# nwihardjo/SpaghettiSearch

Measured on AMD Instinct MI355X. Metric: pagerank_iters_per_sec, higher is better.
Workload: dtype f64

## Files before the change

### include/spaghetti_rank.h

```cpp
#ifndef SPAGHETTI_RANK_H
#define SPAGHETTI_RANK_H

#include <stdint.h>

#ifdef __cplusplus
extern "C" {
#endif

#define SS_ABI_VERSION 4

enum {
    SS_OK = 0,
    SS_ERR_INVALID = 1,
    SS_ERR_NO_DEVICE = 2,
    SS_ERR_HIP = 3,
    SS_ERR_OOM = 4,
    SS_ERR_UNSORTED = 5,
    SS_ERR_STATE = 6,
    SS_ERR_UNSUPPORTED = 7,
    SS_ERR_COMM = 8
};

#define SS_MAX_TOPK 1024
#define SS_MAX_TOPICS 64
#define SS_MAX_QUERY_TERMS 64
#define SS_MAX_CONSTRAINT_TERMS 16
#define SS_UNKNOWN_TERM 0xFFFFFFFFu

typedef struct ss_ctx ss_ctx;
typedef struct ss_graph ss_graph;
typedef struct ss_pr ss_pr;
typedef struct ss_index ss_index;
typedef struct ss_scorer ss_scorer;

typedef struct ss_hit {
    uint32_t doc;
    uint32_t _pad;
    double title;
    double body;
    double pagerank;
    double final;
} ss_hit;

typedef struct ss_graph_info {
    uint64_t n_nodes, n_edges;
    uint64_t n_nondangling;
    uint64_t n_rows_local;
    uint64_t n_edges_local;
    uint32_t max_indeg;
    int32_t rank, world;
} ss_graph_info;

int32_t ss_abi_version(void);
int32_t ss_init(int32_t device_id, ss_ctx** out);
int32_t ss_shutdown(ss_ctx* ctx);
int32_t ss_set_stream(ss_ctx* ctx, void* hip_stream);
int32_t ss_synchronize(ss_ctx* ctx);
#define SS_OPTION_DEFAULT INT64_MIN
int32_t ss_set_option(ss_ctx* ctx, const char* name, int64_t value);
const char* ss_last_error(ss_ctx* ctx);

#define SS_COMM_ID_BYTES 128
int32_t ss_comm_unique_id(void* id_out );
int32_t ss_comm_init(ss_ctx* ctx, const void* id , int32_t rank, int32_t world);
int32_t ss_comm_split(ss_ctx* ctx, int32_t color, int32_t key);
int32_t ss_comm_destroy(ss_ctx* ctx);
int32_t ss_comm_info(ss_ctx* ctx, int32_t* rank_out , int32_t* world_out);
int32_t ss_comm_allreduce_u64(ss_ctx* ctx, uint64_t* buf, uint64_t n);
int32_t ss_comm_allgather(ss_ctx* ctx, const void* send, void* recv, uint64_t bytes_per_rank);

int32_t ss_graph_create(ss_ctx* ctx, uint64_t n_nodes, uint64_t n_edges,
                        const uint64_t* out_ptr , const uint32_t* out_dst ,
                        int32_t rank, int32_t world, ss_graph** out);
int32_t ss_graph_apply_delta(ss_graph* g, uint64_t n_nodes_new, uint64_t n_changed, const uint32_t* changed ,
                             const uint64_t* new_ptr , const uint32_t* new_children);
int32_t ss_graph_get_info(const ss_graph* g, ss_graph_info* info);
int32_t ss_graph_destroy(ss_graph* g);

#define SS_MAX_LINKS      64
#define SS_LINKS_PARENTS  0
#define SS_LINKS_CHILDREN 1
int32_t ss_graph_set_link_key(ss_graph* g, const double* key );
int32_t ss_graph_top_links(ss_graph* g, int32_t dir, uint64_t n, const uint32_t* nodes , int32_t m,
                           uint32_t* links_out , int32_t* n_out , uint32_t* degree_out );
int32_t ss_graph_hit_links(ss_graph* g, int32_t dir, int32_t n_q, int32_t k,
                           const ss_hit* hits , const int32_t* n_hits , int32_t m,
                           uint32_t* links_out , int32_t* n_out ,
                           uint32_t* degree_out );

int32_t ss_pagerank_run(ss_graph* g, double damping, double eps, int32_t max_iter,
                        int32_t k_topics, const int32_t* n_topic,
                        double* rank_out, int32_t* iters_out);

int32_t ss_pr_create(ss_graph* g, double damping, double eps, int32_t max_iter,
                     int32_t k_topics, const int32_t* n_topic, ss_pr** out);
int32_t ss_pr_destroy(ss_pr* pr);
int32_t ss_pr_set_teleport(ss_pr* pr, const uint64_t* set_ptr , const uint32_t* set_nodes);
int32_t ss_pr_begin(ss_pr* pr);
int32_t ss_pr_step(ss_pr* pr, int32_t n_steps);
int32_t ss_pr_lean_sweeps(ss_pr* pr, int64_t* n_out);
int32_t ss_pr_finalize(ss_pr* pr);
int32_t ss_pr_exchange_buffers(ss_pr* pr, void** send_dev, uint64_t* send_bytes,
                               void** recv_dev, uint64_t* recv_bytes);
int32_t ss_pr_exchange(ss_pr* pr, int32_t allreduce);
int32_t ss_pagerank_run_sharded(ss_graph* g, double damping, double eps, int32_t max_iter, int32_t k_topics,
                                const int32_t* n_topic, int32_t allreduce, uint32_t* ids_out, double* rank_out, int32_t* iters_out);
int32_t ss_pagerank_run_group(ss_graph* const* shards, int32_t world, double damping, double eps, int32_t max_iter, int32_t k_topics,
                              const int32_t* n_topic, double* rank_out, int32_t* iters_out);
int32_t ss_pr_status(ss_pr* pr, int32_t* iters_out, int32_t* n_active, int32_t* sweeps,
                     double* last_delta_out , double* last_total_out );
int32_t ss_pr_read_local(ss_pr* pr, uint32_t* ids_out, double* rank_out);
int32_t ss_pr_read(ss_pr* pr, double* rank_out);

int32_t ss_pr_probe(ss_pr* pr, int32_t mode, int32_t n_reps, float* ms_out);

int32_t ss_index_create(ss_ctx* ctx, uint64_t n_docs, uint64_t n_terms,
                        const uint64_t* term_ptr , const uint32_t* post_doc,
                        const float* post_tf, ss_index** out);
int32_t ss_index_destroy(ss_index* idx);
int32_t ss_tfidf_build(ss_index* idx, uint64_t total_docs,
                       float* w_out, double* mag_out, float* idf_out);
int32_t ss_index_set_doc_freq(ss_index* idx, const uint64_t* df );
int32_t ss_index_set_weighted(ss_index* idx, const double* mag );
int32_t ss_index_set_positions(ss_index* idx, const uint64_t* pos_ptr, const float* pos);

int32_t ss_index_apply_delta(ss_index* idx, uint64_t n_del_docs, const uint32_t* del_docs,
                             uint64_t n_del, const uint32_t* del_term, const uint32_t* del_doc,
                             uint64_t n_add, const uint32_t* add_term, const uint32_t* add_doc, const float* add_w);
int32_t ss_index_apply_delta_pos(ss_index* idx, uint64_t n_del_docs, const uint32_t* del_docs,
                                 uint64_t n_del, const uint32_t* del_term, const uint32_t* del_doc,
                                 uint64_t n_add, const uint32_t* add_term, const uint32_t* add_doc, const float* add_w,
                                 const uint64_t* add_pos_ptr , const float* add_pos);
int32_t ss_index_resize(ss_index* idx, uint64_t n_docs_new, uint64_t n_terms_new);
int32_t ss_index_read_magnitudes(ss_index* idx, uint64_t n, const uint32_t* docs, double* mag_out);
int32_t ss_index_refresh_magnitudes(ss_index* idx, double* mag_out);
int32_t ss_index_get_info(const ss_index* idx, uint64_t* n_docs, uint64_t* n_terms, uint64_t* n_post);
int32_t ss_index_read(ss_index* idx, uint64_t* term_ptr_out , uint32_t* post_doc_out, float* post_w_out);
int32_t ss_index_read_positions(ss_index* idx, uint64_t* pos_ptr_out, float* pos_out);

int32_t ss_index_build_doc_view(ss_index* idx);
int32_t ss_index_drop_doc_view(ss_index* idx);
int32_t ss_index_read_doc_view(ss_index* idx, uint64_t* doc_ptr_out, uint32_t* doc_term_out, float* doc_w_out);
int32_t ss_index_doc_top_terms(ss_index* idx, uint64_t n, const uint32_t* docs , int32_t m,
                               uint32_t* terms_out , float* w_out , int32_t* n_out );

int32_t ss_scorer_create(ss_ctx* ctx, ss_index* title, ss_index* body, ss_scorer** out);
int32_t ss_scorer_destroy(ss_scorer* s);
int32_t ss_scorer_set_prior(ss_scorer* s, int32_t k_topics, const double* rank);
int32_t ss_score_topk(ss_scorer* s, int32_t n_q, const uint32_t* q_ptr, const uint32_t* q_terms,
                      const int32_t* query_len, const double* topic_probs, int32_t k,
                      ss_hit* hits_out, int32_t* n_hits_out);

#define SS_SCORE_INFLIGHT 3
int32_t ss_score_topk_submit(ss_scorer* s, int32_t n_q, const uint32_t* q_ptr, const uint32_t* q_terms,
                             const uint32_t* p_ptr ,
                             const uint32_t* p_terms, const int32_t* query_len, const double* topic_probs, int32_t k,
                             uint64_t* ticket_out);
int32_t ss_score_topk_collect(ss_scorer* s, uint64_t ticket, ss_hit* hits_out, int32_t* n_hits_out);

#define SS_MAX_PHRASE_TERMS 16
int32_t ss_score_topk_phrase(ss_scorer* s, int32_t n_q, const uint32_t* q_ptr, const uint32_t* q_terms,
                             const uint32_t* p_ptr, const uint32_t* p_terms, const int32_t* query_len,
                             const double* topic_probs, int32_t k, ss_hit* hits_out, int32_t* n_hits_out);

int32_t ss_scorer_set_doc_masks(ss_scorer* s, int32_t n_masks, const uint32_t* words);

int32_t ss_score_topk_masked(ss_scorer* s, int32_t n_q, const uint32_t* q_ptr, const uint32_t* q_terms,
                             const uint32_t* p_ptr, const uint32_t* p_terms, const int32_t* query_len,
                             const double* topic_probs, const int32_t* mask_id, int32_t k,
                             ss_hit* hits_out, int32_t* n_hits_out);

int32_t ss_score_topk_constrained(ss_scorer* s, int32_t n_q, const uint32_t* q_ptr, const uint32_t* q_terms,
                                  const uint32_t* p_ptr, const uint32_t* p_terms, const int32_t* query_len,
                                  const double* topic_probs, const int32_t* mask_id,
                                  const uint32_t* req_ptr , const uint32_t* req_terms,
                                  const uint32_t* exc_ptr , const uint32_t* exc_terms,
                                  int32_t k, ss_hit* hits_out, int32_t* n_hits_out);

int32_t ss_similar_topk(ss_scorer* s, int32_t n_q, const uint32_t* seeds , int32_t m,
                        const double* topic_probs, const int32_t* mask_id , int32_t k,
                        ss_hit* hits_out, int32_t* n_hits_out);

#define SS_MAX_FEEDBACK_DOCS 64
int32_t ss_related_terms(ss_scorer* s, int32_t n_q, const uint32_t* q_ptr, const uint32_t* q_terms,
                         const int32_t* query_len, const double* topic_probs, const int32_t* mask_id ,
                         int32_t k_fb, int32_t m_doc, int32_t m,
                         uint32_t* terms_out , double* score_out , int32_t* n_out );

typedef struct ss_term_match {
    float    title_w;
    float    body_w;
    uint32_t flags;
    float    body_pos;
} ss_term_match;
int32_t ss_explain_hits(ss_scorer* s, int32_t n_q, const uint32_t* q_ptr, const uint32_t* q_terms,
                        int32_t k, const ss_hit* hits , const int32_t* n_hits ,
                        int32_t t_stride, ss_term_match* out );

typedef struct ss_passage {
    float    start;
    float    last;
    uint32_t n_distinct;
    uint32_t n_occ;
    uint64_t token_mask;
} ss_passage;
int32_t ss_best_passages(ss_scorer* s, int32_t n_q, const uint32_t* q_ptr, const uint32_t* q_terms,
                         int32_t k, const ss_hit* hits , const int32_t* n_hits ,
                         int32_t width, ss_passage* out );

#define SS_NO_GROUP 0xFFFFFFFFu
int32_t ss_scorer_set_doc_groups(ss_scorer* s, const uint32_t* group );

int32_t ss_collapse_hits(ss_scorer* s, int32_t n_q, int32_t k_in, const ss_hit* hits ,
                         const int32_t* n_hits , int32_t g, int32_t first, int32_t k,
                         ss_hit* hits_out , int32_t* n_hits_out ,
                         uint32_t* same_out , int32_t* n_kept_out );

int32_t ss_score_topk_collapsed(ss_scorer* s, int32_t n_q, const uint32_t* q_ptr, const uint32_t* q_terms,
                                const int32_t* query_len, const double* topic_probs, const int32_t* mask_id ,
                                int32_t k_window, int32_t g, int32_t first, int32_t k,
                                ss_hit* hits_out , int32_t* n_hits_out ,
                                uint32_t* same_out , int32_t* n_kept_out );

#define SS_MAX_SIG_SLOTS 32
#define SS_SIG_EMPTY 0xFFFFFFFFu
int32_t ss_index_build_signatures(ss_index* idx, int32_t n_slots);
int32_t ss_index_drop_signatures(ss_index* idx);
int32_t ss_index_read_signatures(ss_index* idx, uint64_t n, const uint32_t* docs ,
                                 uint32_t* sig_out , int32_t* n_slots_out );

int32_t ss_dedup_hits(ss_scorer* s, int32_t n_q, int32_t k_in, const ss_hit* hits , const int32_t* n_hits ,
                      int32_t min_match, int32_t first, int32_t k,
                      ss_hit* hits_out , int32_t* n_hits_out ,
                      uint32_t* similar_out , int32_t* n_kept_out );

#define SS_MAX_DOC_FIELDS 4
#define SS_MAX_RANGE_CLAUSES 4
#define SS_NO_FIELD_VALUE INT64_MIN
typedef struct ss_doc_range {
    int32_t field;
    int32_t _pad;
    int64_t lo, hi;
} ss_doc_range;
int32_t ss_scorer_set_doc_fields(ss_scorer* s, int32_t n_fields, const int64_t* values );

int32_t ss_doc_field_masks(ss_scorer* s, int32_t n_sets, const uint32_t* rng_ptr , const ss_doc_range* rng,
                           const int32_t* mask_id ,
                           uint32_t* words_out );

int32_t ss_score_topk_filtered(ss_scorer* s, int32_t n_q, const uint32_t* q_ptr, const uint32_t* q_terms,
                               const uint32_t* p_ptr, const uint32_t* p_terms, const int32_t* query_len,
                               const double* topic_probs, const int32_t* mask_id,
                               const uint32_t* req_ptr , const uint32_t* req_terms,
// ... 136 lines not shown
```

### spaghettisearch_amd/_lib.py

```python
from __future__ import annotations

import ctypes as C
import os

_HERE = os.path.dirname(os.path.abspath(__file__))
LIB_PATH = os.environ.get("SS_LIB_PATH") or os.path.join(_HERE, "libspaghetti_rank.so")

SS_OK = 0
SS_MAX_TOPK = 1024
SS_MAX_TOPICS = 64
SS_MAX_QUERY_TERMS = 64
SS_MAX_FEEDBACK_DOCS = 64
SS_UNKNOWN_TERM = 0xFFFFFFFF
SS_NO_GROUP = 0xFFFFFFFF
SS_MAX_WORD_BYTES = 64
SS_MAX_EDIT_DIST = 3
SS_MAX_SUGGEST = 64
SS_MAX_COMPLETE = 64
SS_MAX_SIG_SLOTS = 32
SS_SIG_EMPTY = 0xFFFFFFFF
SS_MAX_LINKS = 64
SS_LINKS_PARENTS = 0
SS_LINKS_CHILDREN = 1
SS_MAX_DOC_FIELDS = 4
SS_MAX_RANGE_CLAUSES = 4
SS_NO_FIELD_VALUE = -(2 ** 63)
SS_MAX_VEC_DIM = 1024
SS_NO_VEC_SCORE = -(2 ** 31)
SS_DIV_WEIGHT_MAX = 65536
SS_MAX_VEC_LISTS = 65536
SS_NO_LIST = 0xFFFFFFFF
SS_FUSE_RRF = 0
SS_FUSE_WEIGHTED = 1

ERR_NAMES = {0: "SS_OK", 1: "SS_ERR_INVALID", 2: "SS_ERR_NO_DEVICE", 3: "SS_ERR_HIP", 4: "SS_ERR_OOM",
             5: "SS_ERR_UNSORTED", 6: "SS_ERR_STATE", 7: "SS_ERR_UNSUPPORTED", 8: "SS_ERR_COMM"}
SS_COMM_ID_BYTES = 128


class SpaghettiError(RuntimeError):
    def __init__(self, code: int, msg: str):
        super().__init__(f"{ERR_NAMES.get(code, code)}: {msg}")
        self.code = code


class SsHit(C.Structure):
    _fields_ = [("doc", C.c_uint32), ("_pad", C.c_uint32), ("title", C.c_double), ("body", C.c_double),
                ("pagerank", C.c_double), ("final", C.c_double)]


class SsTermMatch(C.Structure):
    _fields_ = [("title_w", C.c_float), ("body_w", C.c_float), ("flags", C.c_uint32), ("body_pos", C.c_float)]


class SsPassage(C.Structure):
    _fields_ = [("start", C.c_float), ("last", C.c_float), ("n_distinct", C.c_uint32), ("n_occ", C.c_uint32), ("token_mask", C.c_uint64)]


class SsDocRange(C.Structure):
    _fields_ = [("field", C.c_int32), ("_pad", C.c_int32), ("lo", C.c_int64), ("hi", C.c_int64)]


class SsVecHit(C.Structure):
    _fields_ = [("doc", C.c_uint32), ("score", C.c_int32)]


class SsDivInfo(C.Structure):
    _fields_ = [("rel", C.c_int32), ("sim", C.c_int32)]


class SsFuseParams(C.Structure):
    _fields_ = [("mode", C.c_int32), ("rrf_c", C.c_int32), ("w_lex", C.c_double), ("w_vec", C.c_double)]


class SsFused(C.Structure):
    _fields_ = [("score", C.c_double), ("vec_score", C.c_int32), ("lex_rank", C.c_uint16), ("vec_rank", C.c_uint16)]


class SsGraphInfo(C.Structure):
    _fields_ = [("n_nodes", C.c_uint64), ("n_edges", C.c_uint64), ("n_nondangling", C.c_uint64),
                ("n_rows_local", C.c_uint64), ("n_edges_local", C.c_uint64), ("max_indeg", C.c_uint32),
                ("rank", C.c_int32), ("world", C.c_int32)]


_vp = C.c_void_p
_i32 = C.c_int32
_u64 = C.c_uint64
_f64 = C.c_double

PROTOTYPES = {
    "ss_abi_version": (_i32, []),
    "ss_init": (_i32, [_i32, C.POINTER(_vp)]),
    "ss_shutdown": (_i32, [_vp]),
    "ss_set_stream": (_i32, [_vp, _vp]),
    "ss_synchronize": (_i32, [_vp]),
    "ss_set_option": (_i32, [_vp, C.c_char_p, C.c_int64]),
    "ss_last_error": (C.c_char_p, [_vp]),
    "ss_comm_unique_id": (_i32, [_vp]),
    "ss_comm_init": (_i32, [_vp, _vp, _i32, _i32]),
    "ss_comm_split": (_i32, [_vp, _i32, _i32]),
    "ss_comm_destroy": (_i32, [_vp]),
    "ss_comm_info": (_i32, [_vp, C.POINTER(_i32), C.POINTER(_i32)]),
    "ss_comm_allreduce_u64": (_i32, [_vp, _vp, _u64]),
    "ss_comm_allgather": (_i32, [_vp, _vp, _vp, _u64]),
    "ss_graph_create": (_i32, [_vp, _u64, _u64, _vp, _vp, _i32, _i32, C.POINTER(_vp)]),
    "ss_graph_apply_delta": (_i32, [_vp, _u64, _u64, _vp, _vp, _vp]),
    "ss_graph_get_info": (_i32, [_vp, C.POINTER(SsGraphInfo)]),
    "ss_graph_destroy": (_i32, [_vp]),
    "ss_graph_set_link_key": (_i32, [_vp, _vp]),
    "ss_graph_top_links": (_i32, [_vp, _i32, _u64, _vp, _i32, _vp, _vp, _vp]),
    "ss_graph_hit_links": (_i32, [_vp, _i32, _i32, _i32, _vp, _vp, _i32, _vp, _vp, _vp]),
    "ss_pagerank_run": (_i32, [_vp, _f64, _f64, _i32, _i32, _vp, _vp, _vp]),
    "ss_pr_create": (_i32, [_vp, _f64, _f64, _i32, _i32, _vp, C.POINTER(_vp)]),
    "ss_pr_destroy": (_i32, [_vp]),
    "ss_pr_set_teleport": (_i32, [_vp, _vp, _vp]),
    "ss_pr_begin": (_i32, [_vp]),
    "ss_pr_step": (_i32, [_vp, _i32]),
    "ss_pr_lean_sweeps": (_i32, [_vp, C.POINTER(C.c_int64)]),
    "ss_pr_finalize": (_i32, [_vp]),
    "ss_pr_exchange_buffers": (_i32, [_vp, C.POINTER(_vp), C.POINTER(_u64), C.POINTER(_vp), C.POINTER(_u64)]),
    "ss_pr_exchange": (_i32, [_vp, _i32]),
    "ss_pagerank_run_sharded": (_i32, [_vp, _f64, _f64, _i32, _i32, _vp, _i32, _vp, _vp, _vp]),
    "ss_pagerank_run_group": (_i32, [_vp, _i32, _f64, _f64, _i32, _i32, _vp, _vp, _vp]),
    "ss_pr_status": (_i32, [_vp, _vp, C.POINTER(_i32), C.POINTER(_i32), _vp, _vp]),
    "ss_pr_read_local": (_i32, [_vp, _vp, _vp]),
    "ss_pr_read": (_i32, [_vp, _vp]),
    "ss_pr_probe": (_i32, [_vp, _i32, _i32, C.POINTER(C.c_float)]),
    "ss_index_create": (_i32, [_vp, _u64, _u64, _vp, _vp, _vp, C.POINTER(_vp)]),
    "ss_index_destroy": (_i32, [_vp]),
    "ss_tfidf_build": (_i32, [_vp, _u64, _vp, _vp, _vp]),
    "ss_index_apply_delta": (_i32, [_vp, _u64, _vp, _u64, _vp, _vp, _u64, _vp, _vp, _vp]),
    "ss_index_apply_delta_pos": (_i32, [_vp, _u64, _vp, _u64, _vp, _vp, _u64, _vp, _vp, _vp, _vp, _vp]),
    "ss_index_resize": (_i32, [_vp, _u64, _u64]),
    "ss_index_read_magnitudes": (_i32, [_vp, _u64, _vp, _vp]),
    "ss_index_refresh_magnitudes": (_i32, [_vp, _vp]),
    "ss_index_get_info": (_i32, [_vp, C.POINTER(_u64), C.POINTER(_u64), C.POINTER(_u64)]),
    "ss_index_read": (_i32, [_vp, _vp, _vp, _vp]),
    "ss_index_read_positions": (_i32, [_vp, _vp, _vp]),
    "ss_index_set_doc_freq": (_i32, [_vp, _vp]),
    "ss_index_set_weighted": (_i32, [_vp, _vp]),
    "ss_index_set_positions": (_i32, [_vp, _vp, _vp]),
    "ss_index_build_doc_view": (_i32, [_vp]),
    "ss_index_drop_doc_view": (_i32, [_vp]),
    "ss_index_read_doc_view": (_i32, [_vp, _vp, _vp, _vp]),
    "ss_index_doc_top_terms": (_i32, [_vp, _u64, _vp, _i32, _vp, _vp, _vp]),
    "ss_scorer_create": (_i32, [_vp, _vp, _vp, C.POINTER(_vp)]),
    "ss_scorer_destroy": (_i32, [_vp]),
    "ss_scorer_set_prior": (_i32, [_vp, _i32, _vp]),
    "ss_score_topk": (_i32, [_vp, _i32, _vp, _vp, _vp, _vp, _i32, _vp, _vp]),
    "ss_score_topk_phrase": (_i32, [_vp, _i32, _vp, _vp, _vp, _vp, _vp, _vp, _i32, _vp, _vp]),
    "ss_score_topk_submit": (_i32, [_vp, _i32, _vp, _vp, _vp, _vp, _vp, _vp, _i32, _vp]),
    "ss_score_topk_collect": (_i32, [_vp, C.c_uint64, _vp, _vp]),
    "ss_scorer_set_doc_masks": (_i32, [_vp, _i32, _vp]),
    "ss_score_topk_masked": (_i32, [_vp, _i32, _vp, _vp, _vp, _vp, _vp, _vp, _vp, _i32, _vp, _vp]),
    "ss_score_topk_constrained": (_i32, [_vp, _i32, _vp, _vp, _vp, _vp, _vp, _vp, _vp, _vp, _vp, _vp, _vp, _i32, _vp, _vp]),
    "ss_similar_topk": (_i32, [_vp, _i32, _vp, _i32, _vp, _vp, _i32, _vp, _vp]),
    "ss_related_terms": (_i32, [_vp, _i32, _vp, _vp, _vp, _vp, _vp, _i32, _i32, _i32, _vp, _vp, _vp]),
    "ss_explain_hits": (_i32, [_vp, _i32, _vp, _vp, _i32, _vp, _vp, _i32, _vp]),
    "ss_best_passages": (_i32, [_vp, _i32, _vp, _vp, _i32, _vp, _vp, _i32, _vp]),
    "ss_scorer_set_doc_groups": (_i32, [_vp, _vp]),
    "ss_collapse_hits": (_i32, [_vp, _i32, _i32, _vp, _vp, _i32, _i32, _i32, _vp, _vp, _vp, _vp]),
    "ss_score_topk_collapsed": (_i32, [_vp, _i32, _vp, _vp, _vp, _vp, _vp, _i32, _i32, _i32, _i32, _vp, _vp, _vp, _vp]),
    "ss_index_build_signatures": (_i32, [_vp, _i32]),
    "ss_index_drop_signatures": (_i32, [_vp]),
    "ss_index_read_signatures": (_i32, [_vp, _u64, _vp, _vp, C.POINTER(_i32)]),
    "ss_dedup_hits": (_i32, [_vp, _i32, _i32, _vp, _vp, _i32, _i32, _i32, _vp, _vp, _vp, _vp]),
    "ss_scorer_set_doc_fields": (_i32, [_vp, _i32, _vp]),
    "ss_doc_field_masks": (_i32, [_vp, _i32, _vp, _vp, _vp, _vp]),
    "ss_score_topk_filtered": (_i32, [_vp, _i32, _vp, _vp, _vp, _vp, _vp, _vp, _vp, _vp, _vp, _vp, _vp, _vp, _vp, _i32, _vp, _vp]),
    "ss_facet_counts": (_i32, [_vp, _i32, _vp, _vp, _vp, _vp, _vp, _vp, _vp, _vp, _vp, _i32, _vp, _vp, _vp, _vp]),
    "ss_field_topk": (_i32, [_vp, _i32, _vp, _vp, _vp, _vp, _vp, _vp, _vp, _vp, _vp, _i32, _i32, _i32, _i32, _vp, _vp, _vp, _vp]),
    "ss_scorer_group_values": (_i32, [_vp, _vp, _vp]),
    "ss_top_groups": (_i32, [_vp, _i32, _vp, _vp, _vp, _vp, _vp, _vp, _vp, _vp, _vp, _i32, _i32, _vp, _vp, _vp, _vp, _vp]),
    "ss_sort_hits_by_field": (_i32, [_vp, _i32, _i32, _vp, _vp, _i32, _i32, _i32, _i32, _vp, _vp, _vp]),
    "ss_hit_fields": (_i32, [_vp, _i32, _i32, _vp, _vp, _vp]),
    "ss_scorer_set_doc_vectors": (_i32, [_vp, _i32, _vp]),
    "ss_vector_topk": (_i32, [_vp, _i32, _vp, _vp, _i32, _vp, _vp]),
    "ss_hit_vector_scores": (_i32, [_vp, _i32, _vp, _i32, _vp, _vp, _vp]),
    "ss_rerank_hits_by_vector": (_i32, [_vp, _i32, _vp, _i32, _vp, _vp, _i32, _i32, _vp, _vp, _vp]),
    "ss_diversify_hits": (_i32, [_vp, _i32, _vp, _i32, _vp, _vp, _i32, _i32, _i32, _i32, _vp, _vp, _vp]),
    "ss_scorer_set_vector_lists": (_i32, [_vp, _i32, _vp, _vp]),
    "ss_vector_assign_lists": (_i32, [_vp, _i32, _vp, _vp, _vp]),
    "ss_vector_topk_probed": (_i32, [_vp, _i32, _vp, _vp, _i32, _i32, _vp, _vp, _vp]),
    "ss_score_docs": (_i32, [_vp, _i32, _vp, _vp, _vp, _vp, _i32, _vp, _vp, _vp]),
    "ss_fuse_hits": (_i32, [_vp, _i32, _vp, _vp, _vp, _vp, _vp, _i32, _vp, _vp, _i32, _vp, _vp, _vp, _i32, _i32, _vp, _vp, _vp, _vp]),
    "ss_hybrid_topk": (_i32, [_vp, _i32, _vp, _vp, _vp, _vp, _vp, _vp, _i32, _vp, _i32, _i32, _vp, _vp, _vp, _vp]),
    "ss_lexicon_create": (_i32, [_vp, _u64, _vp, _vp, _vp, C.POINTER(_vp)]),
    "ss_lexicon_set_freq": (_i32, [_vp, _vp]),
    "ss_lexicon_get_info": (_i32, [_vp, C.POINTER(_u64), C.POINTER(_u64)]),
    "ss_lexicon_read_order": (_i32, [_vp, _vp]),
    "ss_lexicon_destroy": (_i32, [_vp]),
    "ss_lexicon_prefix": (_i32, [_vp, _i32, _vp, _vp, C.c_int64, _i32, _vp, _vp, _vp]),
    "ss_lexicon_suggest": (_i32, [_vp, _i32, _vp, _vp, _i32, C.c_uint32, _i32, _vp, _vp, _vp]),
    "ss_lexicon_complete": (_i32, [_vp, _i32, _vp, _vp, C.c_uint32, _i32, _vp, _vp, _vp, _vp]),
    "ss_merge_hits": (_i32, [_vp, _i32, _i32, _i32, _vp, _vp, _vp, _vp, _vp]),
    "ss_last_kernel_ms": (_i32, [_vp, _i32, C.POINTER(C.c_float)]),
}

ABI_VERSION = 4
_lib = None


def load() -> C.CDLL:
    global _lib
    if _lib is not None:
        return _lib
    if not os.path.exists(LIB_PATH):
        raise ImportError(
            f"{LIB_PATH} not found: build it with `python -c 'import __graft_entry__ as g; g.build()'` "
            "(make -C spaghettisearch_amd/csrc). There is no CPU fallback.")
    try:
        import torch
    except ImportError:
        pass
    lib = C.CDLL(LIB_PATH)
    for name, (res, args) in PROTOTYPES.items():
        fn = getattr(lib, name)
        fn.restype = res
        fn.argtypes = args
    if lib.ss_abi_version() != ABI_VERSION:
        raise ImportError(f"{LIB_PATH}: ABI version {lib.ss_abi_version()}, this binding was written for {ABI_VERSION} "
                          "(include/spaghetti_rank.h: SS_ABI_VERSION) - rebuild the library")
    _lib = lib
    return lib


def check(rc: int, ctx=None) -> None:
    if rc != SS_OK:
        msg = load().ss_last_error(ctx)
        raise SpaghettiError(rc, msg.decode("utf-8", "replace") if msg else "")
```

### spaghettisearch_amd/csrc/ctx.hip

```cpp
#include "common.hpp"
#include <chrono>

#include <unordered_map>

namespace ss {

namespace {
struct Pool {
    std::mutex mu;
    std::multimap<std::pair<int, size_t>, void*> free_blocks;
    std::unordered_map<void*, std::pair<int, size_t>> live;
    size_t held = 0, limit = (size_t)64 << 30;
    double miss_ms = 0.0;
    uint64_t misses = 0;
    int contexts = 0;
};
Pool& pool() { static Pool* p = new Pool(); return *p; }
size_t size_class(size_t b) {
    if (b <= 4096) return 4096;
    size_t p2 = 4096;
    while (p2 < b) p2 <<= 1;
    if (p2 <= ((size_t)1 << 20)) return p2;
    const size_t step = p2 >> 4;
    return (b + step - 1) / step * step;
// ... 105 lines not shown
        last = delta < 0 && pool().contexts <= 0;
    }
    if (last) pool_trim();
}

void pool_trim() {
    Pool& P = pool();
    std::multimap<std::pair<int, size_t>, void*> take;
    {
        std::lock_guard<std::mutex> lk(P.mu);
        take.swap(P.free_blocks);
        P.held = 0;
    }
    for (auto& kv : take) (void)hipFree(kv.second);
}

void pool_set_limit(size_t bytes) {
    {
        std::lock_guard<std::mutex> lk(pool().mu);
        pool().limit = bytes;
    }
    pool_trim();
}

static std::mutex g_err_mu;
static std::string g_err;
void set_global_error(const std::string& msg) {
    std::lock_guard<std::mutex> lk(g_err_mu);
    g_err = msg;
}
}

extern "C" {

int32_t ss_abi_version(void) { return SS_ABI_VERSION; }

int32_t ss_init(int32_t device_id, ss_ctx** out) {
    if (!out) {
        ss::set_global_error("ss_init: out is NULL");
        return SS_ERR_INVALID;
    }
    *out = nullptr;
    int n_dev = 0;
    hipError_t e = hipGetDeviceCount(&n_dev);
    if (e != hipSuccess || n_dev <= 0) {
        ss::set_global_error(std::string("ss_init: no HIP device (") + hipGetErrorString(e) + ")");
        return SS_ERR_NO_DEVICE;
    }
    if (device_id < 0 || device_id >= n_dev) {
        ss::set_global_error("ss_init: device_id out of range");
        return SS_ERR_INVALID;
    }
    ss_ctx* ctx = new (std::nothrow) ss_ctx();
    if (!ctx) return SS_ERR_OOM;
    ctx->device = device_id;
    if ((e = hipSetDevice(device_id)) != hipSuccess) {
        ss::set_global_error(std::string("ss_init: hipSetDevice: ") + hipGetErrorString(e));
        delete ctx;
        return SS_ERR_NO_DEVICE;
    }
    hipDeviceProp_t prop;
    if ((e = hipGetDeviceProperties(&prop, device_id)) != hipSuccess) {
        ss::set_global_error(std::string("ss_init: hipGetDeviceProperties: ") + hipGetErrorString(e));
        delete ctx;
        return SS_ERR_NO_DEVICE;
    }
    if (std::strncmp(prop.gcnArchName, "gfx950", 6) != 0) {
        ss::set_global_error(std::string("ss_init: device is ") + prop.gcnArchName +
                             ", this library is built for gfx950 (MI355X) only");
        delete ctx;
        return SS_ERR_NO_DEVICE;
    }
    ctx->cu_count = prop.multiProcessorCount;
    ctx->total_mem = prop.totalGlobalMem;
    if ((e = hipStreamCreateWithFlags(&ctx->own_stream, hipStreamNonBlocking)) != hipSuccess) {
        ss::set_global_error(std::string("ss_init: hipStreamCreate: ") + hipGetErrorString(e));
        delete ctx;
        return SS_ERR_HIP;
    }
    ctx->stream = ctx->own_stream;
    int prio_lo = 0, prio_hi = 0;
    (void)hipDeviceGetStreamPriorityRange(&prio_lo, &prio_hi);
    if ((e = hipStreamCreateWithPriority(&ctx->comm_stream, hipStreamNonBlocking, prio_hi)) != hipSuccess) {
        ss::set_global_error(std::string("ss_init: hipStreamCreate (comm): ") + hipGetErrorString(e));
        (void)hipStreamDestroy(ctx->own_stream);
        delete ctx;
        return SS_ERR_HIP;
    }
    for (int k = 0; k < 3; k++)
        for (int j = 0; j < 2; j++)
            if ((e = hipEventCreate(&ctx->ev[k][j])) != hipSuccess) {
                ss::set_global_error(std::string("ss_init: hipEventCreate: ") + hipGetErrorString(e));
                delete ctx;
                return SS_ERR_HIP;
            }
    if ((e = hipHostMalloc(reinterpret_cast<void**>(&ctx->h_pin), ss_ctx::PIN_SCRATCH, hipHostMallocDefault)) != hipSuccess) {
        ss::set_global_error(std::string("ss_init: hipHostMalloc: ") + hipGetErrorString(e));
        delete ctx;
        return SS_ERR_HIP;
    }
    ss::pool_context_count(+1);
    *out = ctx;
    return SS_OK;
}

int32_t ss_shutdown(ss_ctx* ctx) {
    if (!ctx) return SS_ERR_INVALID;
    (void)hipSetDevice(ctx->device);
    const bool stuck = !ss::try_unwedge(ctx);
    (void)ss_comm_destroy(ctx);
    if (!stuck) (void)hipStreamSynchronize(ctx->stream);
    for (int k = 0; k < 3; k++)
        for (int j = 0; j < 2; j++)
            if (ctx->ev[k][j]) (void)hipEventDestroy(ctx->ev[k][j]);
    if (ctx->comm_stream && !stuck) { (void)hipStreamSynchronize(ctx->comm_stream); (void)hipStreamDestroy(ctx->comm_stream); }
    for (hipStream_t ws : ctx->wave_stream)
        if (ws && !stuck) { (void)hipStreamSynchronize(ws); (void)hipStreamDestroy(ws); }
    if (ctx->own_stream && !stuck) (void)hipStreamDestroy(ctx->own_stream);
    if (ctx->h_pin) (void)hipHostFree(ctx->h_pin);
    for (auto& b : ctx->pin_cache) (void)hipHostFree(b.p);
    delete ctx;
    ss::pool_context_count(-1);
    return SS_OK;
}

int32_t ss_set_stream(ss_ctx* ctx, void* hip_stream) {
    if (!ctx) return SS_ERR_INVALID;
    std::lock_guard<std::recursive_mutex> lk(ctx->mu);
    SS_HIP(ctx, hipStreamSynchronize(ctx->stream));
    ctx->stream = hip_stream ? reinterpret_cast<hipStream_t>(hip_stream) : ctx->own_stream;
    return SS_OK;
}

static const char* const k_option_names[] = {
    "comm.timeout_ms",
    "pr.force_narrow",
    "pr.wire_f32",
    "pr.narrow_wave",
    "pr.t_quad",
    "pr.blocks_per_cu",
    "mem.pool_mb",
    "pr.deal_snake",
    "pr.affine_lag",
    "pr.affine",
    "pr.items_per_wave",
    "pr.persistent",
    "pr.persistent_blocks",
    "pr.n_class_order",
    "pr.class_order",
    "pr.stagger",
    "pr.deal_global",
    "pr.share_zero_rows",
    "pr.lean_sweeps",
    "pr.item_turns",
    "graph.late_free",
    "graph.readback_runs",
    "pr.trace",
    "score.collect_pinned",
    "score.pipeline_slices",
    "score.timing",
    "score.trace",
    "pr.probe_hot",
    "pr.topic_blocks",
    "tfidf.blocks",
    "tfidf.bucket_shift",
    "tfidf.head_min_run",
    "tfidf.bucket_min",
    "score.wave",
    "score.wave_max_terms",
    "score.wave_min_list",
    "score.wave_share_pct",
    "score.wave_slice_target",
    "score.wave_big_pct",
    "score.wave_big_x100",
    "score.small",
    "score.small_max_batch",
    "score.small_batch",
    "score.small_cap",
    "score.pipeline",
    "score.grade_slices",
    "score.wave_small_x100",
    "score.exact_all",
    "score.slice_target",
    "score.separate_merge",
    "passage.lds_events",
    "lexicon.chunk_terms",
    "lexicon.complete_parts",
    "links.wave_max",
    "links.chunk_edges",
    "vec.chunk_docs",
    "vec.list_seg_rows",
    "vec.list_batch_q",
    "vec.assign_batch",
    "div.scratch_bytes",
    "ftopk.runs",
    "ftopk.scratch_bytes",
    "gtopk.lds_groups",
    "gtopk.runs",
    "gtopk.scratch_bytes",
};

int32_t ss_set_option(ss_ctx* ctx, const char* name, int64_t value) {
    if (!ctx || !name) return SS_ERR_INVALID;
    std::lock_guard<std::recursive_mutex> lk(ctx->mu);
    for (const char* n : k_option_names)
        if (std::strcmp(n, name) == 0) {
            if (value == SS_OPTION_DEFAULT) ctx->options.erase(name);
            else ctx->options[name] = value;
            if (std::strcmp(name, "mem.pool_mb") == 0) ss::pool_set_limit(value == SS_OPTION_DEFAULT ? (size_t)64 << 30 : (size_t)std::max<int64_t>(0, value) << 20);
            return SS_OK;
        }
    return ctx->fail(SS_ERR_INVALID, "ss_set_option: unknown option '%s'", name);
}

int32_t ss_synchronize(ss_ctx* ctx) {
    if (!ctx) return SS_ERR_INVALID;
    std::lock_guard<std::recursive_mutex> lk(ctx->mu);
    SS_HIP(ctx, hipSetDevice(ctx->device));
    SS_TRY(ss::sync_bounded(ctx, ctx->stream, "ss_synchronize"));
    return SS_OK;
}

const char* ss_last_error(ss_ctx* ctx) {
    if (ctx) return ctx->last_error.c_str();
    static thread_local std::string tl;
    {
        std::lock_guard<std::mutex> lk(ss::g_err_mu);
        tl = ss::g_err;
    }
    return tl.c_str();
}

int32_t ss_last_kernel_ms(ss_ctx* ctx, int32_t kind, float* ms_out) {
    if (!ctx || !ms_out || kind < 0 || kind > 2) return SS_ERR_INVALID;
    std::lock_guard<std::recursive_mutex> lk(ctx->mu);
    if (!ctx->ev_valid[kind]) return ctx->fail(SS_ERR_STATE, "ss_last_kernel_ms: no timed call of kind %d yet", kind);
    SS_HIP(ctx, hipEventSynchronize(ctx->ev[kind][1]));
    SS_HIP(ctx, hipEventElapsedTime(ms_out, ctx->ev[kind][0], ctx->ev[kind][1]));
    return SS_OK;
}

}
```

### spaghettisearch_amd/csrc/pagerank.hip

```cpp
#include "pr_device.hpp"

#include <algorithm>
#include <chrono>
#include <cmath>
#include <memory>

namespace {

__global__ void k_pr_item_ranges(WorkItem* __restrict__ work, uint32_t n_items, const uint32_t* __restrict__ in_ptr) {
    const uint32_t i = blockIdx.x * blockDim.x + threadIdx.x;
    if (i >= n_items) return;
    WorkItem w = work[i];
    switch (w.kind) {
        case V_ROWW: w.beg = in_ptr[w.row]; w.end = in_ptr[w.row + 1]; break;
        case V_SEG:
            w.beg = in_ptr[w.row] + w.count * SEGW;
            w.end = min(in_ptr[w.row + 1], w.beg + SEGW);
            break;
        case V_QUAD:
        case V_DEG: w.beg = in_ptr[w.row]; w.end = in_ptr[w.row + w.count]; break;
        default: return;
    }
    work[i] = w;
}
// ... 96 lines not shown
        int owner;
        if (iid < nd_int) { owner = (int)(iid / sl_nd); lrow = (uint32_t)(iid % sl_nd); }
        else { owner = (int)((iid - nd_int) / sl_d); lrow = sl_nd + (uint32_t)((iid - nd_int) % sl_d); }
        if (owner == rank) atomicOr(&memb[lrow], 1u << k);
    }
}
__global__ void k_pr_memb_zero_count(const uint32_t* __restrict__ memb, uint32_t sl_nd, uint32_t cnt_nd, uint32_t pos_nd, uint32_t cnt_d,
                                     uint32_t pos_d, int k_topics, unsigned long long* __restrict__ cnt) {
    const uint32_t z_nd = cnt_nd - pos_nd, n_zero = z_nd + (cnt_d - pos_d);
    for (uint32_t i = blockIdx.x * blockDim.x + threadIdx.x; i < n_zero; i += gridDim.x * blockDim.x) {
        const uint32_t lrow = i < z_nd ? pos_nd + i : sl_nd + pos_d + (i - z_nd);
        const uint32_t mb = memb[lrow];
        for (int k = 0; k < k_topics; k++)
            if ((mb >> k) & 1u) atomicAdd(&cnt[k], 1ull);
    }
}

template <int GW, int POL>
__global__ __launch_bounds__(TPB) void k_pr_probe(const double* __restrict__ T, const uint32_t* __restrict__ in_src, size_t n_edges,
                                                  uint32_t n_rows, int mode, double* __restrict__ sink, uint32_t hot) {
    if constexpr (GW >= 8) {
        constexpr int NSLOT = 64 / GW;
        const int lane = threadIdx.x & 63, wave = threadIdx.x >> 6;
        const int t = lane % GW, slot = lane / GW, gbase = lane - t;
        const size_t groups = (size_t)gridDim.x * WAVES * NSLOT;
        const size_t gi = ((size_t)blockIdx.x * WAVES + wave) * NSLOT + slot;
        const size_t n_chunks = n_edges / CH;
        const size_t per = (n_chunks + groups - 1) / groups;
        size_t c = min(gi * per, n_chunks);
        const size_t c_hi = min(c + per, n_chunks);
        double acc = 0.0;
        for (; c < c_hi; c++) {
            constexpr int R = CH / GW;
            uint32_t src[R];
#pragma unroll
            for (int r = 0; r < R; r++) {
                const size_t e = c * CH + (size_t)(r * GW + t);
                uint32_t v = NT_LOAD(&in_src[e]) & SRC_MASK;
                if (mode == 1) v = (uint32_t)(((uint64_t)(v * 2654435761u + (uint32_t)e * 40503u) * n_rows) >> 32);
                if (mode == 2) v = (uint32_t)(e % n_rows);
                src[r] = v;
            }
            double v[CH];
#pragma unroll
            for (int j = 0; j < CH; j++) {
                const uint32_t sj = (uint32_t)__shfl((int)src[j / GW], gbase + (j % GW), 64);
                const double* a = &T[(size_t)sj * GW + t];
                if constexpr (POL == 0) v[j] = *a;
                else if constexpr (POL == 1) v[j] = __builtin_nontemporal_load(a);
                else if constexpr (POL == 2) v[j] = __hip_atomic_load(a, __ATOMIC_RELAXED, __HIP_MEMORY_SCOPE_AGENT);
                else if constexpr (POL == 3) v[j] = sj < hot ? *a : __builtin_nontemporal_load(a);
                else v[j] = sj < hot ? *a : __hip_atomic_load(a, __ATOMIC_RELAXED, __HIP_MEMORY_SCOPE_AGENT);
            }
#pragma unroll
            for (int j = 0; j < CH; j++) acc += v[j];
        }
        sink[((size_t)blockIdx.x * TPB + threadIdx.x)] = acc;
    }
}

}

namespace {

void pick_kernel(const ss_ctx* ctx, ss_pr* pr, int k, uint64_t table_rows) {
    const bool force_narrow = ctx->opt("pr.force_narrow", 0) != 0, narrow_wave = ctx->opt("pr.narrow_wave", 1) != 0;
    if (k > 2) {
        pr->kernel = PR_SWEEP;
        pr->gw = k <= 8 ? 8 : 16;
    } else if (force_narrow) {
        pr->kernel = PR_STEP;
        pr->gw = k;
    } else if (narrow_wave) {
        pr->kernel = PR_SWEEP_N;
        pr->gw = k;
    } else if (table_rows * 64 <= (64ull << 20)) {
        pr->kernel = PR_SWEEP;
        pr->gw = 8;
    } else {
        pr->kernel = PR_STEP;
        pr->gw = k;
    }
    pr->nwave = pr->kernel == PR_SWEEP_N;
    const int64_t want = ctx->opt("pr.persistent", 0);
    pr->persist_mode = want == 2 ? 2 : 1;
    pr->persist = pr->nwave && pr->g->world == 1 && !ctx->opt("pr.affine", 0) && want > 0;
}

template <int GW>
void launch_begin(ss_pr* pr, hipStream_t st, unsigned nb) {
    hipLaunchKernelGGL(k_pr_begin<GW>, dim3(nb), dim3(TPB), 0, st, pr->prm);
}
template <int GW>
void launch_finalize(ss_pr* pr, hipStream_t st, int is_begin) {
    hipLaunchKernelGGL(k_pr_finalize<GW>, dim3(1), dim3(64), 0, st, pr->prm, (const double*)pr->tab0.p, is_begin);
}
template <int GW>
__global__ __launch_bounds__(TPB) void k_pr_read_orig(const double* __restrict__ x, const PrCtl* __restrict__ ctl, const uint32_t* __restrict__ new_id,
                                                      uint64_t n, uint32_t sl_nd, uint32_t pos_nd, uint32_t pos_d, int k_topics,
                                                      double* __restrict__ out, const uint32_t* __restrict__ memb, uint32_t ts_mask) {
    const uint64_t v = (uint64_t)blockIdx.x * blockDim.x + threadIdx.x;
    if (v >= n) return;
    const uint32_t lrow = new_id[v];
    const bool zero = lrow < sl_nd ? lrow >= pos_nd : (lrow - sl_nd) >= pos_d;
    double r[GW];
    if (!zero) {
        if constexpr (GW >= 2) {
            const double2* const row = reinterpret_cast<const double2*>(x + (size_t)lrow * GW);
#pragma unroll
            for (int j = 0; j < GW / 2; j++) { const double2 t = row[j]; r[2 * j] = t.x; r[2 * j + 1] = t.y; }
        } else {
            r[0] = x[lrow];
        }
    } else {
        const uint32_t mb = memb ? memb[lrow] & ts_mask : 0u;
#pragma unroll
        for (int k = 0; k < GW; k++) r[k] = ((mb >> k) & 1u) ? ctl->xz_in[k] : ctl->xz[k];
    }
#pragma unroll
    for (int k = 0; k < GW; k++)
        if (k < k_topics) out[(size_t)k * n + v] = r[k];
}

template <int GW>
void launch_read(ss_pr* pr, hipStream_t st, int by_orig, uint64_t stride, uint32_t* ids, double* out) {
    const ss_graph* g = pr->g;
    const size_t n_rows = (size_t)g->cnt_nd + g->cnt_d;
    if (!n_rows) return;
    if (by_orig && g->world == 1 && !ids && stride == g->n) {
        hipLaunchKernelGGL(k_pr_read_orig<GW>, dim3(ss::div_up(g->n, TPB)), dim3(TPB), 0, st, (const double*)pr->x.p, (const PrCtl*)pr->ctl.p,
                           (const uint32_t*)g->new_id.p, g->n, g->sl_nd, pr->prm.pos_nd, pr->prm.pos_d, pr->k, out, pr->prm.memb, pr->prm.ts_mask);
        return;
    }
    hipLaunchKernelGGL(k_pr_read<GW>, dim3(ss::div_up(n_rows, TPB)), dim3(TPB), 0, st, (const double*)pr->x.p,
                       (const PrCtl*)pr->ctl.p, (const uint32_t*)g->old_id.p, g->sl_nd, g->cnt_nd, pr->prm.pos_nd, g->sl_d, g->cnt_d,
                       pr->prm.pos_d,
                       (uint64_t)g->rank * g->sl_nd, g->nd_int + (uint64_t)g->rank * g->sl_d, pr->k, stride, by_orig, ids, out,
                       pr->prm.memb, pr->prm.ts_mask);
}

#define SS_GW_DISPATCH(gw, fn, ...)          \
    switch (gw) {                            \
        case 1: fn<1>(__VA_ARGS__); break;   \
        case 2: fn<2>(__VA_ARGS__); break;   \
        case 8: fn<8>(__VA_ARGS__); break;   \
        default: fn<16>(__VA_ARGS__); break; \
    }

}

namespace ss {
unsigned begin_blocks(const ss_pr* pr) { return std::max(1u, std::min(2048u, ss::div_up((size_t)pr->g->n_local() * pr->gw, TPB))); }
void pr_launch_begin(ss_pr* pr, hipStream_t st, unsigned nb) { SS_GW_DISPATCH(pr->gw, launch_begin, pr, st, nb); }
void pr_launch_step(ss_pr* pr, hipStream_t st, bool lean) {
    switch (pr->kernel) {
        case PR_STEP: pr_step_launch(pr, st); break;
        case PR_SWEEP: pr_sweep_launch(pr, st, lean); break;
        case PR_SWEEP_N: pr_sweep_n_launch(pr, st); break;
    }
}
void pr_launch_finalize(ss_pr* pr, hipStream_t st, int is_begin) { SS_GW_DISPATCH(pr->gw, launch_finalize, pr, st, is_begin); }
}

namespace {

PlanOptions plan_options(const ss_ctx* ctx, const ss_pr* pr, size_t n_local) {
    const bool small = n_local <= ((size_t)4 << 20);
    PlanOptions o;
    o.t_quad = (uint32_t)ctx->opt("pr.t_quad", pr->nwave ? 256 : 128);
    o.item_turns = (uint32_t)std::max<int64_t>(1, std::min<int64_t>(64, ctx->opt("pr.item_turns", pr->nwave ? (small ? 1 : 4) : (small ? 4 : 8))));
    o.items_per_wave = pr->nwave ? (size_t)std::max<int64_t>(1, ctx->opt("pr.items_per_wave", 4)) : 1;
    o.deal_snake = ctx->opt("pr.deal_snake", PlanOptions::AUTO);
    o.deal_global = ctx->opt("pr.deal_global", pr->nwave && pr->gw == 1 ? 1 : 2);
    o.blocks_per_cu = ctx->opt("pr.blocks_per_cu", PlanOptions::AUTO);
    o.class_order = ctx->opt("pr.class_order", 235401);
    o.n_class_order = ctx->opt("pr.n_class_order", small ? 2310 : 123);
    o.stagger = ctx->opt("pr.stagger", 0);
    return o;
}

constexpr int OCC_MULTI_N = 3;
int blocks_per_cu(int row, int gw) {
    static std::mutex occ_mu;
    static int occ_cache[4][MAXK + 1] = {};
    std::lock_guard<std::mutex> lk_occ(occ_mu);
    int& occ = occ_cache[row][gw];
    if (!occ) {
        int per_cu = 0;
        switch (row) {
            case PR_STEP: per_cu = ss::pr_step_occupancy(gw); break;
            case PR_SWEEP: per_cu = ss::pr_sweep_occupancy(gw); break;
            case PR_SWEEP_N: per_cu = ss::pr_sweep_n_occupancy(gw); break;
            default: per_cu = ss::pr_multi_n_occupancy(gw); break;
        }
        occ = std::max(per_cu, 1);
    }
    return occ;
}
unsigned grid_for(const ss_ctx* ctx, const ss_pr* pr, const PlanOptions& opt, int per_cu, size_t n_items) {
    per_cu = (int)std::max<int64_t>(1, opt.blocks_per_cu == PlanOptions::AUTO ? per_cu : opt.blocks_per_cu);
    if (pr->persist) {
        const int admit = std::max(1, blocks_per_cu(OCC_MULTI_N, pr->gw) - 2);
        per_cu = (int)std::max<int64_t>(1, std::min<int64_t>(std::min(admit, std::max(1, per_cu / 2)), ctx->opt("pr.persistent_blocks", 4)));
    }
    return pr->kernel != PR_STEP ? (unsigned)std::min<size_t>(std::max<size_t>(1, ss::div_up(n_items, (size_t)WAVES * opt.items_per_wave)), (size_t)ctx->cu_count * per_cu)
                                 : (unsigned)std::min<size_t>(n_items, (size_t)ctx->cu_count * 8);
}

void fill_params(ss_pr* pr, const Cut& cut, const PlanOptions& opt, double damping, double eps, int32_t max_iter, int32_t k_topics) {
    const ss_graph* g = pr->g;
    PrParams& p = pr->prm;
    p.in_ptr = g->in_ptr.p;
    p.in_src = g->in_src.p;
    p.outdeg = g->outdeg.p;
    p.x = pr->x.p;
    if (g->world == 1) {
        p.tab_rd[0] = pr->tab0.p; p.tab_wr[0] = pr->tab1.p;
        p.tab_rd[1] = pr->tab1.p; p.tab_wr[1] = pr->tab0.p;
    } else {
        p.tab_rd[0] = p.tab_rd[1] = pr->tab0.p;
        p.tab_wr[0] = p.tab_wr[1] = pr->send.p;
    }
    p.work = pr->work.p;
    p.partials = pr->partials.p;
    p.segpart = pr->segpart.p;
    p.rowticket = pr->rowticket.p;
    p.hubsum = pr->hubsum.p;
    p.nmulti = cut.nmulti;
    p.ctl = pr->ctl.p;
    p.x0 = pr->x0.p;
    p.d = damping;
    p.teleport = 1.0 - damping;
    p.eps = eps;
    p.tele_n = p.teleport * (double)g->n;
    p.max_iter = max_iter;
    p.k_topics = k_topics;
    p.world = g->world;
    p.sl_nd = g->sl_nd;
    p.cnt_nd = g->cnt_nd;
    p.sl_d = g->sl_d;
    p.cnt_d = g->cnt_d;
    p.seg_edges = cut.seg_edges;
    p.n_items = (uint32_t)cut.items.size();
    p.pos_nd = cut.pos_nd;
    p.pos_d = cut.pos_d;
    p.zrow = (uint32_t)g->nd_int;
    p.tab_rows = g->sl_nd;
    p.woff = pr->woff.p;
    p.stagger_div = opt.stagger != 0 ? (uint32_t)std::max(g->ctx->cu_count, 1) : 0u;
    p.stagger_code = opt.stagger >= 10 ? (uint32_t)(opt.stagger - 10) : 0u;
    p.class_order = pack_class_order(opt.class_order);
    p.n_order = pack_n_order(opt.n_class_order);
    p.woff_lean = pr->lean ? pr->woff_lean.p : nullptr;
}

uint64_t fnv1a(const void* q, size_t n, uint64_t h = 0xcbf29ce484222325ull) {
    const unsigned char* b = static_cast<const unsigned char*>(q);
    for (size_t i = 0; i < n; i++) { h ^= b[i]; h *= 0x100000001b3ull; }
    return h;
}
void trace_plan(const ss_pr* pr, const std::vector<WorkItem>& work, const std::vector<uint32_t>& woff) {
    const PrParams& p = pr->prm;
    const double sd[] = {p.d, p.teleport, p.eps, p.tele_n};
    const uint32_t su[] = {(uint32_t)p.max_iter, (uint32_t)p.k_topics, (uint32_t)p.world, p.sl_nd, p.cnt_nd, p.sl_d, p.cnt_d, p.seg_edges, p.n_items,
                           p.pos_nd, p.pos_d, p.ts_mask, p.zrow, p.stagger_div, p.stagger_code, p.class_order, p.n_order};
    fprintf(stderr, "[pr trace] plan: work %016llx (%zu items)  woff %016llx  params %016llx  nblocks %u\n",
            (unsigned long long)fnv1a(work.data(), work.size() * sizeof(WorkItem)), work.size(),
            (unsigned long long)fnv1a(woff.data(), woff.size() * sizeof(uint32_t)),
            (unsigned long long)fnv1a(su, sizeof(su), fnv1a(sd, sizeof(sd))), pr->nblocks);
}

int32_t alloc_tables(ss_pr* pr, hipStream_t st, size_t rows) {
    const ss_graph* g = pr->g;
    ss_ctx* ctx = g->ctx;
    const size_t GW = (size_t)pr->gw;
    SS_HIP(ctx, pr->tab0.alloc(rows * GW));
    SS_HIP(ctx, hipMemsetAsync(pr->tab0.p, 0, std::max<size_t>(pr->tab0.bytes(), 8), st));
    if (g->world == 1) {
        SS_HIP(ctx, pr->tab1.alloc(rows * GW));
        SS_HIP(ctx, hipMemsetAsync(pr->tab1.p, 0, std::max<size_t>(pr->tab1.bytes(), 8), st));
    } else {
        SS_HIP(ctx, pr->send.alloc((size_t)g->sl_nd * GW));
        SS_HIP(ctx, hipMemsetAsync(pr->send.p, 0, std::max<size_t>(pr->send.bytes(), 8), st));
    }
    return SS_OK;
}
int32_t unshare_rows(ss_pr* pr, hipStream_t st) {
    if (!pr->prm.share) return SS_OK;
    const ss_graph* g = pr->g;
    SS_HIP(g->ctx, hipStreamSynchronize(st));
    SS_TRY(alloc_tables(pr, st, (size_t)g->nd_int + 1));
    pr->src_shared.release();
    pr->sh_deg.release();
    PrParams& p = pr->prm;
    p.tab_rd[0] = pr->tab0.p; p.tab_wr[0] = pr->tab1.p;
    p.tab_rd[1] = pr->tab1.p; p.tab_wr[1] = pr->tab0.p;
    p.in_src = g->in_src.p;
    p.sh_deg = nullptr;
    p.n_shared = 0;
    p.share = 0;
    p.zrow = (uint32_t)g->nd_int;
    p.tab_rows = g->sl_nd;
    return SS_OK;
}

#ifdef SS_PR_WAVETIME
void dump_wave_loads(const Cut& cut, const std::vector<double>& cost, const std::vector<uint32_t>& owner, uint32_t nw) {
    FILE* f = open_dump("pr_load.csv");
    if (!f) return;
    std::vector<double> wl(nw, 0.0), wcls((size_t)nw * 6, 0.0);
    for (size_t i = 0; i < cut.items.size(); i++) {
        int kc = 0; while (kc < 5 && i >= cut.vbeg[kc + 1]) kc++;
        wl[owner[i]] += cost[i]; wcls[(size_t)owner[i] * 6 + kc] += cost[i];
    }
    fprintf(f, "wave,load,c0,c1,c2,c3,c4,c5\n");
    for (uint32_t w = 0; w < nw; w++) fprintf(f, "%u,%.2f,%.2f,%.2f,%.2f,%.2f,%.2f,%.2f\n", w, wl[w], wcls[(size_t)w * 6], wcls[(size_t)w * 6 + 1], wcls[(size_t)w * 6 + 2], wcls[(size_t)w * 6 + 3], wcls[(size_t)w * 6 + 4], wcls[(size_t)w * 6 + 5]);
    fclose(f);
}
#endif

}

extern "C" {

int32_t ss_pr_create(ss_graph* g, double damping, double eps, int32_t max_iter, int32_t k_topics,
                     const int32_t* n_topic, ss_pr** out) {
    if (!g) return SS_ERR_INVALID;
    ss_ctx* ctx = g->ctx;
    std::lock_guard<std::recursive_mutex> lk(ctx->mu);
    if (!out) return ctx->fail(SS_ERR_INVALID, "ss_pr_create: out is NULL");
    *out = nullptr;
    if (k_topics < 1 || !n_topic) return ctx->fail(SS_ERR_INVALID, "ss_pr_create: k_topics < 1 or n_topic NULL");
    if (k_topics > MAXK) return ctx->fail(SS_ERR_UNSUPPORTED, "ss_pr_create: k_topics %d > %d per state (ss_pagerank_run splits larger K)", k_topics, MAXK);
    SS_HIP(ctx, hipSetDevice(ctx->device));
    hipStream_t st = ctx->stream;

    ss_pr* pr = new (std::nothrow) ss_pr();
    if (!pr) return ctx->fail(SS_ERR_OOM, "ss_pr_create: host OOM");
    std::unique_ptr<ss_pr> guard(pr);
    pr->g = g;
    pr->k = k_topics;
    pick_kernel(ctx, pr, k_topics, g->nd_int);
    const int GW = pr->gw;
    const bool vitems = pr->kernel != PR_STEP;
    const int GI = pr->nwave ? 8 : GW;
    const size_t n_local = g->n_local();
    if (((uint64_t)g->nd_int + 1) * GW * 8 >= (1ull << 32))
        return ctx->fail(SS_ERR_UNSUPPORTED, "ss_pr_create: contribution table of %llu rows x %d topics exceeds 4 GiB (shard the graph over more ranks)",
                         (unsigned long long)g->nd_int, GW);

    const bool trace = ctx->opt("pr.trace", 0) != 0;
    auto t_now = [] { return std::chrono::steady_clock::now(); };
    auto t_ms = [](std::chrono::steady_clock::time_point a, std::chrono::steady_clock::time_point b) { return std::chrono::duration<double, std::milli>(b - a).count(); };
    SS_HIP(ctx, pr->x.alloc(n_local * GW));
    bool share = GW >= 8 && g->world == 1 && ctx->opt("pr.affine", 0) == 0 && ctx->opt("pr.share_zero_rows", 1) != 0;
    if (!share) SS_TRY(alloc_tables(pr, st, (size_t)g->nd_int + 1));

    const auto tc0 = t_now();
    const PlanOptions opt = plan_options(ctx, pr, n_local);
    Cut cut = cut_items(g->h_indeg_nd, g->h_indeg_d, g->sl_nd, GI, pr->nwave, opt);
    const uint32_t n_tail = g->cnt_nd - cut.pos_nd;
    struct PinGuard { ss_ctx* c; void* p = nullptr; size_t cap = 0; ~PinGuard() { c->pin_free(p, cap); } } tail_od{ctx};
    if (share && n_tail == 0) {
        share = false;
        SS_TRY(alloc_tables(pr, st, (size_t)g->nd_int + 1));
    }
    if (share) {
        tail_od.p = ctx->pin_alloc((size_t)n_tail * sizeof(uint32_t), &tail_od.cap);
        if (!tail_od.p) return ctx->fail(SS_ERR_OOM, "ss_pr_create: no pinned host memory for %u out-degrees", n_tail);
        SS_HIP(ctx, hipMemcpyAsync(tail_od.p, g->outdeg.p + cut.pos_nd, (size_t)n_tail * sizeof(uint32_t), hipMemcpyDeviceToHost, st));
    }
    const auto tc1 = t_now();
    const int per_cu = blocks_per_cu(pr->kernel, GW);
    const auto tc1a = t_now();
    pr->nblocks = grid_for(ctx, pr, opt, per_cu, cut.items.size());
    static const std::vector<uint32_t> no_woff;
    const std::vector<uint32_t>* woff = &no_woff;
    if (vitems) {
        const uint32_t nw = pr->nblocks * WAVES;
        const auto td0 = t_now();
        const std::vector<double>& cost = item_costs(cut, g->h_indeg_nd, g->h_indeg_d, g->sl_nd, GI, pr->nwave);
        const auto td0a = t_now();
        std::vector<uint32_t>& owner = deal_items(cut, cost, nw, pr->nwave, opt);
#ifdef SS_PR_WAVETIME
        dump_wave_loads(cut, cost, owner, nw);
#endif
        const auto td1 = t_now();
        if (trace) fprintf(stderr, "[pr trace]   deal: occupancy query %.2f ms, costs %.3f ms, owners %.3f ms\n", t_ms(tc1, tc1a), t_ms(td0, td0a), t_ms(td0a, td1));
        woff = &place_items(cut, owner, nw);
        if (trace) fprintf(stderr, "[pr trace]   deal: placement %.3f ms\n", t_ms(td1, t_now()));
    }
    const std::vector<WorkItem>& items = cut.items;
    pr->lean = pr->kernel == PR_SWEEP && g->world == 1 && ctx->opt("pr.affine", 0) == 0 && ctx->opt("pr.lean_sweeps", 1) != 0;
    static const std::vector<WorkItem> no_items;
    const std::vector<WorkItem>* lean_items = &no_items;
    const std::vector<uint32_t>* lean_woff = &no_woff;
    if (pr->lean) {
        const auto tl0 = t_now();
        const LeanPlan lp = plan_lean_items(items, *woff, pr->nblocks * WAVES, g->sl_nd, (uint32_t)items.size());
        lean_items = &lp.items;
        lean_woff = &lp.woff;
        if (trace) fprintf(stderr, "[pr trace]   lean walk: %zu of %zu items, %.3f ms\n", lp.items.size() - 2, items.size() - 2, t_ms(tl0, t_now()));
    }

    g->settle();
    const auto tc2 = t_now();
    SharedRows sh;
    if (share) {
        SS_HIP(ctx, hipStreamSynchronize(st));
        const auto ts0 = t_now();
        sh = plan_shared_rows(static_cast<const uint32_t*>(tail_od.p), n_tail, cut.pos_nd);
        const auto ts1 = t_now();
        SS_TRY(alloc_tables(pr, st, (size_t)sh.table_rows));
        SS_HIP(ctx, pr->sh_deg.alloc(sh.deg.size()));
        SS_HIP(ctx, hipMemcpyAsync(pr->sh_deg.p, sh.deg.data(), sh.deg.size() * sizeof(uint32_t), hipMemcpyHostToDevice, st));
        SS_HIP(ctx, pr->src_shared.alloc(g->e_local));
        if (g->e_local)
            hipLaunchKernelGGL(k_pr_remap_src, dim3((unsigned)std::min<uint64_t>(ss::div_up(g->e_local, TPB), (uint64_t)ctx->cu_count * 16)), dim3(TPB), 0, st,
                               (const uint32_t*)g->in_src.p, pr->src_shared.p, (size_t)g->e_local, cut.pos_nd, g->cnt_nd, (const uint32_t*)g->outdeg.p,
                               (const uint32_t*)pr->sh_deg.p, (uint32_t)sh.deg.size(), sh.zrow);
        if (trace) fprintf(stderr, "[pr trace]   shared rows: %u rows without in-edges -> %zu shared rows (host %.3f ms), table %llu rows\n", n_tail, sh.deg.size(),
                           t_ms(ts0, ts1), (unsigned long long)sh.table_rows);
    }
    SS_HIP(ctx, pr->partials.alloc(((size_t)std::max(pr->nblocks, ss::begin_blocks(pr)) + 8) * 2 * GW));
    SS_HIP(ctx, pr->segpart.alloc((size_t)std::max(cut.nsegs, 1u) * GW));
    SS_HIP(ctx, pr->rowticket.alloc(std::max(cut.nmulti, 1u)));
    SS_HIP(ctx, pr->hubsum.alloc((size_t)std::max(cut.nmulti, 1u) * 2 * GW));
    SS_HIP(ctx, hipMemsetAsync(pr->hubsum.p, 0, pr->hubsum.bytes(), st));
    SS_HIP(ctx, hipMemsetAsync(pr->rowticket.p, 0, pr->rowticket.bytes(), st));
    SS_HIP(ctx, pr->woff.alloc(std::max<size_t>(woff->size(), 8)));
    if (!woff->empty()) SS_HIP(ctx, hipMemcpyAsync(pr->woff.p, woff->data(), woff->size() * sizeof(uint32_t), hipMemcpyHostToDevice, st));
    const size_t n_work = items.size() + lean_items->size();
    SS_HIP(ctx, pr->work.alloc(n_work));
    SS_HIP(ctx, hipMemcpyAsync(pr->work.p, items.data(), items.size() * sizeof(WorkItem), hipMemcpyHostToDevice, st));
    if (pr->lean) {
        SS_HIP(ctx, hipMemcpyAsync(pr->work.p + items.size(), lean_items->data(), lean_items->size() * sizeof(WorkItem), hipMemcpyHostToDevice, st));
        SS_HIP(ctx, pr->woff_lean.alloc(std::max<size_t>(lean_woff->size(), 8)));
        SS_HIP(ctx, hipMemcpyAsync(pr->woff_lean.p, lean_woff->data(), lean_woff->size() * sizeof(uint32_t), hipMemcpyHostToDevice, st));
    }
    if (vitems)
        hipLaunchKernelGGL(k_pr_item_ranges, dim3(ss::div_up(n_work, TPB)), dim3(TPB), 0, st, pr->work.p, (uint32_t)n_work, (const uint32_t*)g->in_ptr.p);
    SS_HIP(ctx, pr->ctl.alloc(1));
    SS_HIP(ctx, hipMemsetAsync(pr->ctl.p, 0, sizeof(PrCtl), st));
    double h_x0[MAXK];
    for (int k = 0; k < MAXK; k++) h_x0[k] = k < k_topics ? 1.0 / (double)n_topic[k] : 0.0;
    SS_HIP(ctx, pr->x0.alloc(MAXK));
    SS_HIP(ctx, hipMemcpyAsync(pr->x0.p, h_x0, sizeof(h_x0), hipMemcpyHostToDevice, st));
    SS_HIP(ctx, hipStreamSynchronize(st));
    if (trace) fprintf(stderr, "[pr trace] ss_pr_create: build_work %.2f ms (%zu items), edge ranges + deal %.2f ms, alloc + upload %.2f ms\n", t_ms(tc0, tc1), items.size(), t_ms(tc1, tc2), t_ms(tc2, t_now()));
    if (trace) fprintf(stderr, "[pr trace] where the state lives: x %p  tab0 %p  tab1 %p  in_src %p  in_ptr %p  outdeg %p  work %p  woff %p\n", (void*)pr->x.p, (void*)pr->tab0.p,
                       (void*)pr->tab1.p, (void*)g->in_src.p, (void*)g->in_ptr.p, (void*)g->outdeg.p, (void*)pr->work.p, (void*)pr->woff.p);

    fill_params(pr, cut, opt, damping, eps, max_iter, k_topics);
    if (share) {
        PrParams& p = pr->prm;
        p.in_src = pr->src_shared.p;
        p.sh_deg = pr->sh_deg.p;
        p.n_shared = (uint32_t)sh.deg.size();
        p.share = 1;
        p.zrow = sh.zrow;
        p.tab_rows = cut.pos_nd;
    }
    if (trace) trace_plan(pr, items, *woff);
    g->users++;
    *out = guard.release();
    return SS_OK;
}

int32_t ss_pr_set_teleport(ss_pr* pr, const uint64_t* set_ptr, const uint32_t* set_nodes) {
    if (!pr) return SS_ERR_INVALID;
    ss_ctx* ctx = pr->g->ctx;
    std::lock_guard<std::recursive_mutex> lk(ctx->mu);
    SS_HIP(ctx, hipSetDevice(ctx->device));
    if (pr->begun) return ctx->fail(SS_ERR_STATE, "ss_pr_set_teleport: call before ss_pr_begin");
    hipStream_t st = ctx->stream;
    PrParams& p = pr->prm;
    if (!set_ptr) {
        p.memb = nullptr; p.tin = nullptr; p.nz_in = nullptr; p.ts_mask = 0;
        return SS_OK;
    }
    const ss_graph* g = pr->g;
    const int K = pr->k;
    SS_TRY(unshare_rows(pr, st));
    std::vector<uint64_t> h_ptr(K + 1);
    SS_HIP(ctx, ss::copy_in(ctx->stream, h_ptr.data(), set_ptr, (K + 1) * sizeof(uint64_t)));
    if (h_ptr[0] != 0) return ctx->fail(SS_ERR_INVALID, "ss_pr_set_teleport: set_ptr[0] != 0");
    for (int k = 0; k < K; k++)
        if (h_ptr[k + 1] < h_ptr[k]) return ctx->fail(SS_ERR_INVALID, "ss_pr_set_teleport: set_ptr not non-decreasing");
    const uint64_t total = h_ptr[K];
    if (total && !set_nodes) return ctx->fail(SS_ERR_INVALID, "ss_pr_set_teleport: set_nodes is NULL");
    double h_tin[MAXK];
    uint32_t mask = 0;
    for (int k = 0; k < MAXK; k++) {
        h_tin[k] = 0.0;
        if (k < K && h_ptr[k + 1] > h_ptr[k]) {
            mask |= 1u << k;
            h_tin[k] = p.teleport * (double)g->n / (double)(h_ptr[k + 1] - h_ptr[k]);
        }
    }
    const size_t n_local = g->n_local();
    ss::DevBuf<uint64_t> d_ptr;
    ss::DevBuf<uint32_t> d_nodes, d_err, d_seen;
    ss::DevBuf<unsigned long long> d_cnt;
    SS_HIP(ctx, d_ptr.alloc(K + 1));
    SS_HIP(ctx, d_seen.alloc(g->n));
    SS_HIP(ctx, hipMemsetAsync(d_seen.p, 0, std::max<size_t>(d_seen.bytes(), 4), st));
    SS_HIP(ctx, d_nodes.alloc(total));
    SS_HIP(ctx, d_err.alloc(1));
    SS_HIP(ctx, d_cnt.alloc(MAXK));
    SS_HIP(ctx, pr->memb.alloc(n_local));
    SS_HIP(ctx, pr->tin.alloc(MAXK));
    SS_HIP(ctx, pr->nz_in.alloc(MAXK));
    SS_HIP(ctx, hipMemcpyAsync(d_ptr.p, h_ptr.data(), (K + 1) * sizeof(uint64_t), hipMemcpyHostToDevice, st));
    if (total) SS_HIP(ctx, hipMemcpyAsync(d_nodes.p, set_nodes, total * sizeof(uint32_t), hipMemcpyDefault, st));
    SS_HIP(ctx, hipMemsetAsync(pr->memb.p, 0, std::max<size_t>(pr->memb.bytes(), 4), st));
    SS_HIP(ctx, hipMemsetAsync(d_err.p, 0, sizeof(uint32_t), st));
    SS_HIP(ctx, hipMemsetAsync(d_cnt.p, 0, MAXK * sizeof(unsigned long long), st));
    if (total)
        hipLaunchKernelGGL(k_pr_memb, dim3(std::min<unsigned>(ss::div_up(total, TPB), 4096u)), dim3(TPB), 0, st, (const uint64_t*)d_ptr.p,
                           (const uint32_t*)d_nodes.p, K, g->n, (const uint32_t*)g->new_id.p, g->nd_int, std::max(g->sl_nd, 1u), std::max(g->sl_d, 1u),
                           g->rank, pr->memb.p, d_seen.p, d_err.p);
    const uint32_t n_zero = (g->cnt_nd - p.pos_nd) + (g->cnt_d - p.pos_d);
    if (n_zero)
        hipLaunchKernelGGL(k_pr_memb_zero_count, dim3(std::min<unsigned>(ss::div_up(n_zero, TPB), 4096u)), dim3(TPB), 0, st,
                           (const uint32_t*)pr->memb.p, g->sl_nd, g->cnt_nd, p.pos_nd, g->cnt_d, p.pos_d, K, d_cnt.p);
    SS_HIP(ctx, hipGetLastError());
    uint32_t h_err = 0;
    unsigned long long h_cnt[MAXK];
    SS_HIP(ctx, ss::fetch(ctx, st, &h_err, d_err.p, sizeof(h_err), h_cnt, d_cnt.p, sizeof(h_cnt)));
    if (h_err & 1u) return ctx->fail(SS_ERR_INVALID, "ss_pr_set_teleport: a teleport set holds a node id >= n_nodes");
    if (h_err & 2u) return ctx->fail(SS_ERR_INVALID, "ss_pr_set_teleport: a teleport set lists a node twice (the ids of a set must be distinct)");
    double h_nz[MAXK];
    for (int k = 0; k < MAXK; k++) h_nz[k] = (double)h_cnt[k];
    SS_HIP(ctx, hipMemcpyAsync(pr->tin.p, h_tin, sizeof(h_tin), hipMemcpyHostToDevice, st));
    SS_HIP(ctx, hipMemcpyAsync(pr->nz_in.p, h_nz, sizeof(h_nz), hipMemcpyHostToDevice, st));
    SS_HIP(ctx, hipStreamSynchronize(st));
    p.memb = pr->memb.p;
    p.tin = pr->tin.p;
    p.nz_in = pr->nz_in.p;
    p.ts_mask = mask;
    return SS_OK;
}

int32_t ss_pr_destroy(ss_pr* pr) {
#ifdef SS_PR_WAVETIME
    if (pr) ss::pr_dump_wave_times(pr);
#endif

    if (!pr) return SS_ERR_INVALID;
    ss_ctx* ctx = pr->g->ctx;
    std::lock_guard<std::recursive_mutex> lk(ctx->mu);
    (void)hipSetDevice(ctx->device);
    if (!ss::device_wedged(ctx->device)) {
        (void)hipStreamSynchronize(ctx->stream);
        (void)hipStreamSynchronize(ctx->comm_stream);
    }
    pr->g->users--;
    delete pr;
    return SS_OK;
}

int32_t ss_pr_begin(ss_pr* pr) {
    if (!pr) return SS_ERR_INVALID;
    ss_ctx* ctx = pr->g->ctx;
    std::lock_guard<std::recursive_mutex> lk(ctx->mu);
    SS_HIP(ctx, hipSetDevice(ctx->device));
    if (pr->need_finalize) return ctx->fail(SS_ERR_STATE, "ss_pr_begin: pending exchange/finalize");
    SS_HIP(ctx, hipMemsetAsync(&pr->ctl.p->ticket, 0, sizeof(uint32_t), ctx->stream));
    ss::pr_launch_begin(pr, ctx->stream, ss::begin_blocks(pr));
    SS_HIP(ctx, hipGetLastError());
    pr->begun = true;
    pr->sweeps_enq = 0;
    if (pr->g->world > 1) {
        pr->need_finalize = true;
        pr->finalize_is_begin = true;
    }
    return SS_OK;
}

int32_t ss_pr_step(ss_pr* pr, int32_t n_steps) {
    if (!pr) return SS_ERR_INVALID;
    return ss::pr_step(pr, n_steps, 2);
}

int32_t ss_pr_lean_sweeps(ss_pr* pr, int64_t* n_out) {
    if (!pr || !n_out) return SS_ERR_INVALID;
    std::lock_guard<std::recursive_mutex> lk(pr->g->ctx->mu);
    *n_out = pr->n_lean;
    return SS_OK;
}

}

int32_t ss::pr_step(ss_pr* pr, int32_t n_steps, int32_t full_tail) {
    ss_ctx* ctx = pr->g->ctx;
    std::lock_guard<std::recursive_mutex> lk(ctx->mu);
    SS_HIP(ctx, hipSetDevice(ctx->device));
    if (!pr->begun) return ctx->fail(SS_ERR_STATE, "ss_pr_step: ss_pr_begin not called");
    if (pr->need_finalize) return ctx->fail(SS_ERR_STATE, "ss_pr_step: pending exchange/finalize");
    if (n_steps < 1) return ctx->fail(SS_ERR_INVALID, "ss_pr_step: n_steps < 1");
    if (pr->g->world > 1 && n_steps != 1) return ctx->fail(SS_ERR_INVALID, "ss_pr_step: world>1 needs an exchange after every step");
    SS_HIP(ctx, hipEventRecord(ctx->ev[0][0], ctx->stream));
    if (pr->persist && !pr->prm.memb && !pr->prm.aff) {
        ss::pr_multi_n_launch(pr, ctx->stream, (int)n_steps);
    } else {
        const PrParams& p = pr->prm;
        const bool lean_ok = pr->lean && p.eps < 0.0 && !p.memb && !p.aff;
        for (int i = 0; i < n_steps; i++) {
            const int64_t s = pr->sweeps_enq + 1 + i;
            const bool lean = lean_ok && i + full_tail < n_steps && (p.max_iter <= 0 || s + 2 <= p.max_iter);
            ss::pr_launch_step(pr, ctx->stream, lean);
        }
    }
    pr->sweeps_enq += n_steps;
    SS_HIP(ctx, hipEventRecord(ctx->ev[0][1], ctx->stream));
    ctx->ev_valid[0] = true;
    SS_HIP(ctx, hipGetLastError());
    if (pr->g->world > 1) {
        pr->need_finalize = true;
        pr->finalize_is_begin = false;
    }
    return SS_OK;
}

extern "C" {

int32_t ss_pr_finalize(ss_pr* pr) {
    if (!pr) return SS_ERR_INVALID;
    ss_ctx* ctx = pr->g->ctx;
    std::lock_guard<std::recursive_mutex> lk(ctx->mu);
    SS_HIP(ctx, hipSetDevice(ctx->device));
    if (pr->g->world == 1) return ctx->fail(SS_ERR_STATE, "ss_pr_finalize: world==1 folds the finalize into the sweep");
    if (!pr->need_finalize) return ctx->fail(SS_ERR_STATE, "ss_pr_finalize: nothing to finalize");
    ss::pr_launch_finalize(pr, ctx->stream, pr->finalize_is_begin ? 1 : 0);
    SS_HIP(ctx, hipGetLastError());
    pr->need_finalize = false;
    return SS_OK;
}

int32_t ss_pr_exchange_buffers(ss_pr* pr, void** send_dev, uint64_t* send_bytes, void** recv_dev, uint64_t* recv_bytes) {
    if (!pr) return SS_ERR_INVALID;
    ss_ctx* ctx = pr->g->ctx;
    if (pr->g->world == 1) return ctx->fail(SS_ERR_STATE, "ss_pr_exchange_buffers: world==1 has no exchange");
    if (send_dev) *send_dev = pr->send.p;
    if (send_bytes) *send_bytes = pr->send.bytes();
    if (recv_dev) *recv_dev = pr->tab0.p;
    if (recv_bytes) *recv_bytes = (uint64_t)pr->g->nd_int * pr->gw * sizeof(double);
    return SS_OK;
}

int32_t ss_pr_exchange(ss_pr* pr, int32_t allreduce) {
    if (!pr) return SS_ERR_INVALID;
    ss_ctx* ctx = pr->g->ctx;
    std::lock_guard<std::recursive_mutex> lk(ctx->mu);
    SS_HIP(ctx, hipSetDevice(ctx->device));
    const ss_graph* g = pr->g;
    if (g->world == 1) return ctx->fail(SS_ERR_STATE, "ss_pr_exchange: world==1 has no exchange");
    if (!pr->need_finalize) return ctx->fail(SS_ERR_STATE, "ss_pr_exchange: nothing to exchange (call after ss_pr_begin / ss_pr_step)");
    if (!ctx->comm || ctx->comm_world != g->world || ctx->comm_rank != g->rank)
        return ctx->fail(SS_ERR_STATE, "ss_pr_exchange: the context's communicator (rank %d of %d) does not match the graph's shard (rank %d of %d)",
                         ctx->comm ? ctx->comm_rank : -1, ctx->comm ? ctx->comm_world : 0, g->rank, g->world);
    const size_t slice = (size_t)g->sl_nd * pr->gw;
    if (!allreduce && ctx->opt("pr.wire_f32", 0) != 0) {
        SS_HIP(ctx, ss::pr_wire_alloc(pr));
        ss::pr_wire_pack(pr, ctx->stream);
        SS_TRY(ss::comm_allgather(ctx, pr->wire_send.p, pr->wire_recv.p, ss::pr_wire_floats(pr) * sizeof(float)));
        ss::pr_wire_unpack(pr, ctx->stream);
        return SS_OK;
    }
    if (!allreduce) return ss::comm_allgather(ctx, pr->send.p, pr->tab0.p, slice * sizeof(double));
    SS_HIP(ctx, hipMemsetAsync(pr->tab0.p, 0, pr->tab0.bytes(), ctx->stream));
    SS_HIP(ctx, hipMemcpyAsync(pr->tab0.p + (size_t)g->rank * slice, pr->send.p, slice * sizeof(double), hipMemcpyDeviceToDevice, ctx->stream));
    return ss::comm_allreduce_f64(ctx, pr->tab0.p, pr->tab0.p, slice * (size_t)g->world);
}

int32_t ss_pr_status(ss_pr* pr, int32_t* iters_out, int32_t* n_active, int32_t* sweeps, double* last_delta_out,
                     double* last_total_out) {
    if (!pr) return SS_ERR_INVALID;
    ss_ctx* ctx = pr->g->ctx;
    std::lock_guard<std::recursive_mutex> lk(ctx->mu);
    SS_HIP(ctx, hipSetDevice(ctx->device));
    const PrCtl* hp = nullptr;
    SS_TRY(read_ctl(ctx, pr, ctx->stream, "ss_pr_status", &hp));
    const PrCtl h = *hp;
    if (h.stuck) return ctx->fail(SS_ERR_STATE, "ss_pr_status: the multi-sweep kernel gave up waiting between two sweeps (its grid of %u blocks was not resident: "
                                  "other kernels held the CUs for seconds); the state is void — set option pr.persistent = 0 and run again", pr->nblocks);
    for (int k = 0; k < pr->k; k++) {
        if (iters_out) iters_out[k] = h.iters[k];
        if (last_delta_out) last_delta_out[k] = h.delta[k];
        if (last_total_out) last_total_out[k] = h.S[k];
    }
    if (n_active) *n_active = h.n_active;
    if (sweeps) *sweeps = h.sweep;
    return SS_OK;
}

int32_t ss_pr_read_local(ss_pr* pr, uint32_t* ids_out, double* rank_out) {
    if (!pr || !rank_out) return SS_ERR_INVALID;
    ss_ctx* ctx = pr->g->ctx;
    std::lock_guard<std::recursive_mutex> lk(ctx->mu);
    SS_HIP(ctx, hipSetDevice(ctx->device));
    const ss_graph* g = pr->g;
    const size_t n_rows = (size_t)g->cnt_nd + g->cnt_d;
    ss::DevBuf<uint32_t> d_ids;
    ss::DevBuf<double> d_out;
    SS_HIP(ctx, d_ids.alloc(n_rows));
    SS_HIP(ctx, d_out.alloc(n_rows * pr->k));
    SS_GW_DISPATCH(pr->gw, launch_read, pr, ctx->stream, 0, (uint64_t)n_rows, d_ids.p, d_out.p);
    SS_HIP(ctx, hipGetLastError());
    if (ids_out && n_rows) SS_HIP(ctx, hipMemcpyAsync(ids_out, d_ids.p, n_rows * sizeof(uint32_t), hipMemcpyDefault, ctx->stream));
    if (n_rows) SS_HIP(ctx, hipMemcpyAsync(rank_out, d_out.p, n_rows * pr->k * sizeof(double), hipMemcpyDefault, ctx->stream));
    SS_HIP(ctx, hipStreamSynchronize(ctx->stream));
    return SS_OK;
}

int32_t ss_pr_read(ss_pr* pr, double* rank_out) {
    if (!pr || !rank_out) return SS_ERR_INVALID;
    ss_ctx* ctx = pr->g->ctx;
    std::lock_guard<std::recursive_mutex> lk(ctx->mu);
    SS_HIP(ctx, hipSetDevice(ctx->device));
    const ss_graph* g = pr->g;
    if (g->world != 1) return ctx->fail(SS_ERR_STATE, "ss_pr_read: world>1, use ss_pr_read_local");
    hipPointerAttribute_t pa{};
    const bool dev_out = hipPointerGetAttributes(&pa, rank_out) == hipSuccess && pa.type == hipMemoryTypeDevice;
    (void)hipGetLastError();
    ss::DevBuf<double> d_out;
    if (!dev_out) SS_HIP(ctx, d_out.alloc((size_t)g->n * pr->k));
    SS_GW_DISPATCH(pr->gw, launch_read, pr, ctx->stream, 1, (uint64_t)g->n, (uint32_t*)nullptr, dev_out ? rank_out : d_out.p);
    SS_HIP(ctx, hipGetLastError());
    if (!dev_out) SS_HIP(ctx, hipMemcpyAsync(rank_out, d_out.p, (size_t)g->n * pr->k * sizeof(double), hipMemcpyDefault, ctx->stream));
    SS_HIP(ctx, hipStreamSynchronize(ctx->stream));
    return SS_OK;
}

int32_t ss_pr_probe(ss_pr* pr, int32_t mode, int32_t n_reps, float* ms_out) {
    if (!pr || !ms_out) return SS_ERR_INVALID;
    ss_ctx* ctx = pr->g->ctx;
    std::lock_guard<std::recursive_mutex> lk(ctx->mu);
    SS_HIP(ctx, hipSetDevice(ctx->device));
    if (pr->gw < 8) return ctx->fail(SS_ERR_UNSUPPORTED, "ss_pr_probe: the probe mirrors the chunked gather of the K >= 5 kernels");
    if (mode < 0 || (mode & 7) > 2 || (mode >> 3) > 4 || n_reps < 1) return ctx->fail(SS_ERR_INVALID, "ss_pr_probe: mode 0..2 (+ 8 * gather cache policy 0..4), n_reps >= 1");
    const int pol = mode >> 3;
    mode &= 7;
    const uint32_t hot = (uint32_t)ctx->opt("pr.probe_hot", 24576);
    const ss_graph* g = pr->g;
    const unsigned nb = (unsigned)ctx->cu_count * 8;
    ss::DevBuf<double> sink;
    SS_HIP(ctx, sink.alloc((size_t)nb * TPB));
    hipEvent_t e0, e1;
    SS_HIP(ctx, hipEventCreate(&e0));
    SS_HIP(ctx, hipEventCreate(&e1));
    hipStream_t st = ctx->stream;
    ss::DevBuf<double> full;
    if (pr->prm.share) {
        SS_HIP(ctx, full.alloc(((size_t)g->nd_int + 1) * pr->gw));
        SS_HIP(ctx, hipMemsetAsync(full.p, 0, full.bytes(), ctx->stream));
    }
    const double* T = pr->prm.share ? full.p : pr->tab0.p;
    for (int r = 0; r < n_reps + 1; r++) {
        if (r == 1) SS_HIP(ctx, hipEventRecord(e0, st));
#define SS_PROBE_LAUNCH(GWV, POLV) hipLaunchKernelGGL((k_pr_probe<GWV, POLV>), dim3(nb), dim3(TPB), 0, st, T, (const uint32_t*)g->in_src.p, (size_t)g->e_local, (uint32_t)g->nd_int, mode, sink.p, hot)
        if (pr->gw == 8) SS_PROBE_LAUNCH(8, 0);
        else switch (pol) {
            case 0: SS_PROBE_LAUNCH(16, 0); break;
// ... 19 lines not shown
```

### spaghettisearch_amd/csrc/pr_device.hpp

```cpp
#pragma once
#include "pr_state.hpp"

#include <cmath>

namespace {


template <int GW>
__device__ __forceinline__ double wave_sum_topic(double v) {
#pragma unroll
    for (int off = GW; off < 64; off <<= 1) v += __shfl_xor(v, off, 64);
    return v;
}

__device__ __forceinline__ double zero_row_rank(const PrParams& p, int sweep, double S, double x0) {
    return ((sweep == 0 ? x0 : 0.0) + p.teleport) / S;
}
__device__ __forceinline__ double teleport_of(const PrParams& p, uint32_t lrow, int t) {
    if (!p.memb || !((p.ts_mask >> t) & 1u)) return p.teleport;
    return ((p.memb[lrow] >> t) & 1u) ? p.tin[t] : 0.0;
}
__device__ __forceinline__ double zero_row_rank_ts(const PrParams& p, int sweep, double S, double x0, double tele) {
    return ((sweep == 0 ? x0 : 0.0) + tele) / S;
}
// ... 88 lines not shown
            } else {
                const double xz = zero_row_rank(p, sw, Sk, p.x0[k]);
                ctl_st<PS>(&ctl->xz[k], xz);
                ctl_st<PS>(&ctl->xz_in[k], xz);
            }
            bool cont = dl[k] > p.eps;
            if (p.max_iter > 0 && it >= p.max_iter) cont = false;
            ctl_st<PS>(&ctl->active[k], cont ? 1 : 0);
            na += cont ? 1 : 0;
            ctl_st<PS>(&ctl->S[k], cs[k] + p.tele_n);
            ctl_st<PS>(&ctl->csum[k], cs[k]);
        }
    }
    ctl_st<PS>(&ctl->n_active, na);
    if constexpr (PS) {
        asm volatile("s_waitcnt vmcnt(0)" ::: "memory");
    }
    ctl_st<PS>(&ctl->sweep, it);
}

template <int GW, int PS = 0>
__device__ __forceinline__ void block_reduce_and_publish(const PrParams& p, double dsum, double csum, double* tail,
                                                         bool is_begin) {
    __shared__ double red[WAVES][2][MAXK];
    __shared__ double tot[2][MAXK];
    __shared__ double colsum[TPB];
    __shared__ int s_last;
    const int lane = threadIdx.x & 63, wave = threadIdx.x >> 6;
    const int t = lane % GW;
    dsum = wave_sum_topic<GW>(dsum);
    csum = wave_sum_topic<GW>(csum);
    if (lane < GW) {
        red[wave][0][t] = dsum;
        red[wave][1][t] = csum;
    }
    __syncthreads();
    if (threadIdx.x < 2 * GW) {
        const int which = threadIdx.x / GW, tt = threadIdx.x % GW;
        double v = red[0][which][tt];
#pragma unroll
        for (int w = 1; w < WAVES; w++) v += red[w][which][tt];
        __hip_atomic_store(&p.partials[(size_t)blockIdx.x * 2 * GW + threadIdx.x], v, __ATOMIC_RELAXED, __HIP_MEMORY_SCOPE_AGENT);
    }
    asm volatile("s_waitcnt vmcnt(0)" ::: "memory");
    __syncthreads();
    constexpr unsigned NG = 8;
    constexpr int NCOL = 2 * GW;
    constexpr int NPART = TPB / NCOL;
    const unsigned ng = min(NG, gridDim.x);
    const unsigned grp = blockIdx.x % ng;
    const unsigned members = (gridDim.x - grp + ng - 1) / ng;
    double* const gpart = p.partials + (size_t)gridDim.x * NCOL;
    if (threadIdx.x == 0) {
        if constexpr (PS == 2) {
            __builtin_amdgcn_fence(__ATOMIC_RELEASE, "agent");
            asm volatile("s_waitcnt vmcnt(0)" ::: "memory");
        }
        const unsigned prev = __hip_atomic_fetch_add(&p.ctl->gticket[grp], 1u, __ATOMIC_RELAXED, __HIP_MEMORY_SCOPE_AGENT);
        s_last = prev == members - 1;
    }
    __syncthreads();
    if (!s_last) return;
    const int col = threadIdx.x % NCOL, part = threadIdx.x / NCOL;
    {
        double acc = 0.0;
        for (unsigned m0 = part; m0 < members; m0 += 16 * NPART) {
            double v[16];
#pragma unroll
            for (int u = 0; u < 16; u++) {
                const unsigned m = m0 + u * NPART;
                v[u] = __hip_atomic_load(&p.partials[(size_t)(grp + ng * (m < members ? m : m0)) * NCOL + col], __ATOMIC_RELAXED, __HIP_MEMORY_SCOPE_AGENT);
            }
#pragma unroll
            for (int u = 0; u < 16; u++)
                if (m0 + u * NPART < members) acc += v[u];
        }
        colsum[threadIdx.x] = acc;
    }
    __syncthreads();
    if (threadIdx.x < NCOL) {
        double v = 0.0;
        for (int q = 0; q < NPART; q++) v += colsum[q * NCOL + threadIdx.x];
        __hip_atomic_store(&gpart[(size_t)grp * NCOL + threadIdx.x], v, __ATOMIC_RELAXED, __HIP_MEMORY_SCOPE_AGENT);
    }
    if (threadIdx.x == 0) ctl_st<PS>(&p.ctl->gticket[grp], 0u);
    asm volatile("s_waitcnt vmcnt(0)" ::: "memory");
    __syncthreads();
    if (threadIdx.x == 0) {
        const unsigned prev = __hip_atomic_fetch_add(&p.ctl->ticket, 1u, __ATOMIC_RELAXED, __HIP_MEMORY_SCOPE_AGENT);
        s_last = prev == ng - 1;
    }
    __syncthreads();
    if (!s_last) return;
    if (threadIdx.x < NCOL) {
        double v = 0.0;
        for (unsigned gq = 0; gq < ng; gq++)
            v += __hip_atomic_load(&gpart[(size_t)gq * NCOL + threadIdx.x], __ATOMIC_RELAXED, __HIP_MEMORY_SCOPE_AGENT);
        tot[threadIdx.x / GW][threadIdx.x % GW] = v;
    } else if (!is_begin && p.nmulti) {
        const unsigned hp = threadIdx.x / NCOL - 1;
        double acc = 0.0;
        for (unsigned h0 = hp; h0 < p.nmulti; h0 += 16 * (NPART - 1)) {
            double v[16];
#pragma unroll
            for (int u = 0; u < 16; u++) {
                const unsigned h = h0 + u * (NPART - 1);
                v[u] = __hip_atomic_load(&p.hubsum[(size_t)(h < p.nmulti ? h : h0) * NCOL + col], __ATOMIC_RELAXED, __HIP_MEMORY_SCOPE_AGENT);
            }
#pragma unroll
            for (int u = 0; u < 16; u++)
                if (h0 + u * (NPART - 1) < p.nmulti) acc += v[u];
        }
        colsum[threadIdx.x] = acc;
    }
    __syncthreads();
    if (!is_begin && p.nmulti && threadIdx.x < NCOL) {
        double v = tot[threadIdx.x / GW][threadIdx.x % GW];
        for (int q = 1; q < NPART; q++) v += colsum[q * NCOL + threadIdx.x];
        tot[threadIdx.x / GW][threadIdx.x % GW] = v;
    }
    __syncthreads();
    if (!is_begin && threadIdx.x < GW && ctl_ld<PS>(&p.ctl->active[threadIdx.x])) {
        const double n_zero = (double)((p.cnt_nd - p.pos_nd) + (p.cnt_d - p.pos_d));
        if (p.memb && ((p.ts_mask >> threadIdx.x) & 1u)) {
            const int k = threadIdx.x;
            const double out_new = zero_row_rank_ts(p, ctl_ld<PS>(&p.ctl->sweep), ctl_ld<PS>(&p.ctl->S[k]), p.x0[k], 0.0);
            const double in_new = zero_row_rank_ts(p, ctl_ld<PS>(&p.ctl->sweep), ctl_ld<PS>(&p.ctl->S[k]), p.x0[k], p.tin[k]);
            tot[0][k] += (n_zero - p.nz_in[k]) * fabs(out_new - ctl_ld<PS>(&p.ctl->xz[k])) + p.nz_in[k] * fabs(in_new - ctl_ld<PS>(&p.ctl->xz_in[k]));
        } else {
            const double xz_new = zero_row_rank(p, ctl_ld<PS>(&p.ctl->sweep), ctl_ld<PS>(&p.ctl->S[threadIdx.x]), p.x0[threadIdx.x]);
            tot[0][threadIdx.x] += n_zero * fabs(xz_new - ctl_ld<PS>(&p.ctl->xz[threadIdx.x]));
        }
    }
    __syncthreads();
    if (p.world == 1) {
        if (threadIdx.x == 0) {
            double dl[MAXK], cs[MAXK];
            for (int k = 0; k < MAXK; k++) {
                dl[k] = k < GW ? tot[0][k] : 0.0;
                cs[k] = k < GW ? tot[1][k] : 0.0;
            }
            ctl_st<PS>(&p.ctl->ticket, 0u);
            finalize_ctl<PS>(p, dl, cs, is_begin);
        }
    } else {
        if (threadIdx.x < GW) {
            tail[(size_t)(p.sl_nd - 2) * GW + threadIdx.x] = tot[1][threadIdx.x];
            tail[(size_t)(p.sl_nd - 1) * GW + threadIdx.x] = tot[0][threadIdx.x];
        }
        if (threadIdx.x == 0) p.ctl->ticket = 0;
    }
}

template <int GA, int GB>
__device__ __attribute__((used, noinline)) void begin_caller_context(const PrParams& p, double* tail) {
    if (!__builtin_constant_p(p.world)) return;
    block_reduce_and_publish<GA>(p, 0.0, 0.0, tail, true);
    block_reduce_and_publish<GB>(p, 0.0, 0.0, tail, true);
}

#define NT_LOAD(p) __builtin_nontemporal_load(p)
#define NT_STORE(v, p) __builtin_nontemporal_store(v, p)

constexpr uint32_t SRC_MASK = 0x7FFFFFFFu;

}
```

### spaghettisearch_amd/csrc/pr_plan.hpp

```cpp
#pragma once
#include "sorted_degrees.hpp"

#include <algorithm>
#include <cstdint>
#include <utility>
#include <vector>

namespace {

constexpr int TPB = 256;
constexpr int WAVES = TPB / 64;
constexpr int CH = 16;
constexpr uint32_t SEGW = 2048;

enum : uint32_t { W_SEG = 0, W_WAVE = 1, W_GROUP = 2, W_ZERO = 3,
                  V_SEG = 8,
                  V_ROWW = 9,
                  V_QUAD = 10,
                  V_DEG = 11,
                  V_ZERO = 12 };

struct WorkItem {
    uint32_t kind;
    uint32_t row;
// ... 200 lines not shown
    auto& load = s.load;
    auto& key = s.key;
    owner.assign(n_items, 0u);
    load.assign(nw, 0.0);
    by_load.resize(nw);
    for (uint32_t w = 0; w < nw; w++) by_load[w] = w;
    const bool snake = (opt.deal_snake == PlanOptions::AUTO ? (n_items >= (size_t)8 * nw || lane_rows ? 1 : 0) : opt.deal_snake) != 0;
    const int64_t deal_mode = opt.deal_global;
    const bool global_order = deal_mode != 0;
    if (global_order) {
        constexpr uint32_t NB = 1u << 14;
        const auto bkey = [&](size_t i) { return NB - 1 - (uint32_t)std::min<double>(cost[i] * 16.0, (double)(NB - 1)); };
        bucket.assign(NB + 1, 0u);
        order.resize(n_items);
        size_t c0 = 0;
        for (int kcls = 0; kcls < (deal_mode == 2 ? 6 : 1); kcls++) {
            const size_t c1 = deal_mode == 2 ? (kcls < 5 ? std::min<size_t>(cut.vbeg[kcls + 1], n_items) : n_items) : n_items;
            if (kcls) std::fill(bucket.begin(), bucket.end(), 0u);
            for (size_t i = c0; i < c1; i++) bucket[bkey(i) + 1]++;
            for (uint32_t b = 0; b < NB; b++) bucket[b + 1] += bucket[b];
            for (size_t i = c0; i < c1; i++) order[c0 + bucket[bkey(i)]++] = (uint32_t)i;
            c0 = c1;
        }
    }
    for (size_t i0 = 0; i0 < n_items; i0 += nw) {
        const size_t n_chunk = std::min<size_t>(nw, n_items - i0);
        if (i0 && snake) {
            std::reverse(by_load.begin(), by_load.end());
        } else if (i0) {
            key.resize(nw);
            for (uint32_t w = 0; w < nw; w++) key[w] = {load[w], w};
            std::sort(key.begin(), key.end());
            for (uint32_t w = 0; w < nw; w++) by_load[w] = key[w].second;
        }
        idx.resize(n_chunk);
        for (size_t j = 0; j < n_chunk; j++) idx[j] = global_order ? order[i0 + j] : (uint32_t)(i0 + j);
        const auto falling = [&](uint32_t a, uint32_t b) { return cost[a] > cost[b]; };
        size_t run_end = 0, n_merge = 0;
        for (size_t j = 1; j <= n_chunk && !global_order; j++) {
            if (j < n_chunk && !(cost[i0 + j] > cost[i0 + j - 1])) continue;
            if (run_end) {
                if (++n_merge > 8) { std::stable_sort(idx.begin(), idx.end(), falling); break; }
                std::inplace_merge(idx.begin(), idx.begin() + (ptrdiff_t)run_end, idx.begin() + (ptrdiff_t)j, falling);
            }
            run_end = j;
        }
        for (size_t j = 0; j < n_chunk; j++) {
            owner[idx[j]] = by_load[j];
            load[by_load[j]] += cost[idx[j]];
        }
    }
    return owner;
}

inline const std::vector<uint32_t>& place_items(Cut& cut, std::vector<uint32_t>& owner, uint32_t nw) {
    PlanScratch& s = plan_scratch();
    auto& items = cut.items;
    auto &woff = s.woff, &cnt = s.cnt;
    woff.assign((size_t)nw * 8, 0);
    cnt.assign((size_t)nw * 8, 0);
    for (int k = 0; k < 6; k++) {
        const size_t i1 = k < 5 ? std::min<size_t>(cut.vbeg[k + 1], items.size()) : items.size();
        for (size_t i = std::min<size_t>(cut.vbeg[k], i1); i < i1; i++) { owner[i] = owner[i] * 8 + (uint32_t)k; cnt[owner[i]]++; }
    }
    uint32_t run_off = 0;
    for (uint32_t w = 0; w < nw; w++) {
        for (int k = 0; k < 8; k++) {
            woff[(size_t)w * 8 + k] = run_off;
            run_off += cnt[(size_t)w * 8 + k];
            cnt[(size_t)w * 8 + k] = woff[(size_t)w * 8 + k];
        }
    }
    s.dealt.resize(items.size());
    for (size_t i = 0; i < items.size(); i++) s.dealt[cnt[owner[i]]++] = items[i];
    s.dealt.push_back({V_ZERO, 0, 0, 0, 0, 0, 0, 0});
    s.dealt.push_back({V_ZERO, 0, 0, 0, 0, 0, 0, 0});
    items.swap(s.dealt);
    return woff;
}

struct LeanPlan {
    const std::vector<WorkItem>& items;
    const std::vector<uint32_t>& woff;
};
inline LeanPlan plan_lean_items(const std::vector<WorkItem>& dealt, const std::vector<uint32_t>& woff, uint32_t nw, uint32_t sl_nd, uint32_t base) {
    PlanScratch& s = plan_scratch();
    auto& items = s.lean_items;
    auto& loff = s.lean_woff;
    items.clear();
    loff.assign((size_t)nw * 8, base);
    const size_t n = dealt.size() >= 2 ? dealt.size() - 2 : 0;
    for (size_t j = 0; j < (size_t)nw * 8 && j < woff.size(); j++) {
        loff[j] = base + (uint32_t)items.size();
        const size_t lo = std::min<size_t>(woff[j], n), hi = j + 1 < woff.size() ? std::min<size_t>(woff[j + 1], n) : n;
        for (size_t i = lo; i < hi; i++)
            if (dealt[i].row < sl_nd) items.push_back(dealt[i]);
    }
    items.push_back({V_ZERO, 0, 0, 0, 0, 0, 0, 0});
    items.push_back({V_ZERO, 0, 0, 0, 0, 0, 0, 0});
    return {items, loff};
}

inline uint32_t pack_class_order(int64_t code) {
    uint32_t packed = 0, seen = 0;
    for (int pos = 5; pos >= 0; pos--) {
        const uint32_t c = (uint32_t)(code % 10);
        code /= 10;
        packed |= (c & 7u) << (3 * pos);
        if (c < 6) seen |= 1u << c;
    }
    return seen == 0x3Fu ? packed : (0u | 1u << 3 | 2u << 6 | 3u << 9 | 4u << 12 | 5u << 15);
}
inline uint32_t pack_n_order(int64_t code) {
    uint32_t packed = 0, seen = 0;
    for (int pos = 3; pos >= 0; pos--) {
        const uint32_t c = (uint32_t)(code % 10);
        code /= 10;
        packed |= (c & 3u) << (2 * pos);
        if (c < 4) seen |= 1u << c;
    }
    return seen == 0xFu ? packed : (0u | 1u << 2 | 2u << 4 | 3u << 6);
}

struct SharedRows {
    std::vector<uint32_t> deg;
    uint32_t zrow = 0;
    uint32_t base = 0;
    uint64_t table_rows = 0;
    uint32_t row_of(uint32_t od) const {
        const auto it = std::lower_bound(deg.begin(), deg.end(), od);
        return it != deg.end() && *it == od ? base + (uint32_t)(it - deg.begin()) : zrow;
    }
};
inline SharedRows plan_shared_rows(const uint32_t* od, size_t n, uint32_t pos_nd) {
    SharedRows sh;
    uint32_t hi = 0;
    for (size_t i = 0; i < n; i++) hi = std::max(hi, od[i]);
    if (n && (uint64_t)hi <= 4 * (uint64_t)n + 65536) {
        std::vector<unsigned char> seen((size_t)hi + 1, 0);
        for (size_t i = 0; i < n; i++) seen[od[i]] = 1;
        for (size_t v = 0; v <= hi; v++)
            if (seen[v]) sh.deg.push_back((uint32_t)v);
    } else if (n) {
        sh.deg.assign(od, od + n);
        std::sort(sh.deg.begin(), sh.deg.end());
        sh.deg.erase(std::unique(sh.deg.begin(), sh.deg.end()), sh.deg.end());
    }
    sh.zrow = pos_nd;
    sh.base = pos_nd + 1;
    sh.table_rows = (uint64_t)pos_nd + 1 + sh.deg.size();
    return sh;
}

}
```

### spaghettisearch_amd/csrc/pr_state.hpp

```cpp
#pragma once
#include "graph.hpp"
#include "pr_plan.hpp"

#ifdef SS_PR_WAVETIME
#include <cstdio>
#include <cstdlib>
#include <string>
#endif

namespace {

constexpr int MAXK = 16;

struct PrCtl {
    double S[MAXK];
    double delta[MAXK];
    double csum[MAXK];
    double xz[MAXK];
    double xz_in[MAXK];
    double tele[MAXK];
    int32_t active[MAXK];
    int32_t iters[MAXK];
    int32_t sweep;
    int32_t n_active;
    uint32_t ticket;
    uint32_t stuck;
    uint32_t gticket[8];
};

constexpr int AFF_MAXK = 256;
constexpr unsigned AFF_NB = 512;
struct AffCtl {
    double u[AFF_MAXK];
    double delta[AFF_MAXK];
    int32_t active[AFF_MAXK], iters[AFF_MAXK], just[AFF_MAXK];
    double r_x, r_prev, r_next;
    double s_x, s_prev, s_next;
    double xz_prev[2];
    int32_t n_active, n_just, k_real, it;
};

struct PrParams {
    const uint32_t* in_ptr;
    const uint32_t* in_src;
    const uint32_t* outdeg;
    double* x;
    const double* tab_rd[2];
    double* tab_wr[2];
    const WorkItem* work;
    double* partials;
    double* segpart;
    uint32_t* rowticket;
    double* hubsum;
    uint32_t nmulti;
    PrCtl* ctl;
    const double* x0;
    double d, teleport, eps, tele_n;
    int32_t max_iter, k_topics, world;
    uint32_t sl_nd, cnt_nd, sl_d, cnt_d, seg_edges, n_items;
    uint32_t pos_nd, pos_d;
    const uint32_t* memb;
    const double* tin;
    const double* nz_in;
    uint32_t ts_mask;
    uint32_t zrow;
    const uint32_t* woff;
    uint32_t stagger_div;
    uint32_t stagger_code;
    uint32_t class_order;
    uint32_t n_order;
    double* x_alt;
    AffCtl* aff;
    const double* tele_col;
    const uint32_t* sh_deg;
    uint32_t n_shared;
    uint32_t share;
    uint32_t tab_rows;
    const uint32_t* woff_lean;
};

}

enum PrKernel : int {
    PR_STEP = 0,
    PR_SWEEP = 1,
    PR_SWEEP_N = 2,
};

struct ss_pr {
    ss_graph* g = nullptr;
    PrKernel kernel = PR_SWEEP;
    int gw = 1;
    ss::DevBuf<float> wire_send, wire_recv;
    bool nwave = false;
    int persist_mode = 1;
    bool persist = false;
    int k = 1;
    PrParams prm{};
    unsigned nblocks = 0;
    ss::DevBuf<double> x, tab0, tab1, send, partials, segpart, hubsum, x0;
    ss::DevBuf<uint32_t> rowticket;
    ss::DevBuf<uint32_t> memb;
    ss::DevBuf<double> tin, nz_in;
    ss::DevBuf<WorkItem> work;
    ss::DevBuf<uint32_t> woff;
    ss::DevBuf<uint32_t> src_shared;
    ss::DevBuf<uint32_t> sh_deg;
    ss::DevBuf<uint32_t> woff_lean;
    bool lean = false;
    int64_t sweeps_enq = 0;
    int64_t n_lean = 0;
    ss::DevBuf<PrCtl> ctl;
    bool begun = false;
    bool need_finalize = false;
    bool finalize_is_begin = false;
};

#pragma GCC visibility push(hidden)
namespace ss {
unsigned begin_blocks(const ss_pr* pr);
void pr_launch_begin(ss_pr* pr, hipStream_t st, unsigned nb);
void pr_launch_step(ss_pr* pr, hipStream_t st, bool lean = false);
int32_t pr_step(ss_pr* pr, int32_t n_steps, int32_t full_tail);
void pr_launch_finalize(ss_pr* pr, hipStream_t st, int is_begin);
void pr_sweep_launch(ss_pr* pr, hipStream_t st, bool lean);
int pr_sweep_occupancy(int gw);
void pr_sweep_n_launch(ss_pr* pr, hipStream_t st);
int pr_sweep_n_occupancy(int gw);
void pr_multi_n_launch(ss_pr* pr, hipStream_t st, int n_steps);
int pr_multi_n_occupancy(int gw);
void pr_step_launch(ss_pr* pr, hipStream_t st);
int pr_step_occupancy(int gw);
#ifdef SS_PR_WAVETIME
void pr_dump_wave_times(const ss_pr* pr);
#endif
size_t pr_wire_floats(const ss_pr* pr);
hipError_t pr_wire_alloc(ss_pr* pr);
void pr_wire_pack(ss_pr* pr, hipStream_t st);
void pr_wire_unpack(ss_pr* pr, hipStream_t st);
}
#pragma GCC visibility pop

namespace {
#ifdef SS_PR_WAVETIME
inline FILE* open_dump(const char* name) {
    const char* dir = getenv("SS_PR_WAVETIME_DIR");
    return fopen((std::string(dir && *dir ? dir : ".") + "/" + name).c_str(), "w");
}
#endif
inline int32_t read_ctl(ss_ctx* ctx, const ss_pr* pr, hipStream_t st, const char* what, const PrCtl** out) {
    ctx->pin_used = 0;
    PrCtl* const hp = ctx->pin<PrCtl>();
    if (hipMemcpyAsync(hp, pr->ctl.p, sizeof(PrCtl), hipMemcpyDeviceToHost, st) != hipSuccess) return ctx->fail(SS_ERR_HIP, "%s: status read failed", what);
    SS_TRY(ss::sync_bounded(ctx, st, what));
    *out = hp;
    return SS_OK;
}
}
```

### spaghettisearch_amd/csrc/pr_sweep.hip

```cpp
#include "pr_device.hpp"

#include <algorithm>

namespace {

template <int GW>
__device__ __forceinline__ double tab_at(const double* __restrict__ T, uint32_t row, int t) {
    return *reinterpret_cast<const double*>(reinterpret_cast<const char*>(T) + (size_t)((row * (uint32_t)GW + (uint32_t)t) * 8u));
}


template <int GW, bool TS, bool LEAN>
struct SweepCtx {
    const PrParams& p;
    const double* __restrict__ T;
    double* __restrict__ Tw;
    double S, x0;
    bool act;
    int t, gbase, slot;
    double dsum, csum;
};

__device__ __forceinline__ uint32_t turn_fill(uint32_t epos, uint32_t lim) {
    return min((uint32_t)CH, __builtin_elementwise_sub_sat(lim, epos));
}

template <int GW>
__device__ __forceinline__ void idx_turn(const uint32_t* __restrict__ in_src, uint32_t epos, uint32_t n, uint32_t zrow, int t, uint32_t (&src)[CH / GW]) {
#pragma unroll
    for (int r = 0; r < CH / GW; r++) {
        const uint32_t j = (uint32_t)(r * GW + t);
        const uint32_t raw = NT_LOAD(&in_src[j < n ? epos + j : 0u]);
        src[r] = j < n ? (raw & SRC_MASK) : zrow;
    }
}
template <int GW>
__device__ __forceinline__ void gather_turn(const double* __restrict__ T, const uint32_t (&src)[CH / GW], int t, int gbase, double (&v)[CH]) {
#pragma unroll
    for (int j = 0; j < CH; j++) {
        const uint32_t sj = (uint32_t)__shfl((int)src[j / GW], gbase + (j % GW), 64);
        v[j] = tab_at<GW>(T, sj, t);
    }
}

template <int GW, bool TS, bool LEAN>
__device__ __forceinline__ void finish_row(SweepCtx<GW, TS, LEAN>& c, uint32_t lrow, double y, double xo, uint32_t od, double* hub = nullptr) {
    const PrParams& p = c.p;
    y += c.x0;
    const size_t xi = (size_t)lrow * GW + c.t;
    double tele = p.teleport;
    if constexpr (TS) tele = teleport_of(p, lrow, c.t);
    double xn = (y + tele) / c.S;
    if constexpr (LEAN) {
        if (!c.act) xn = 0.0;
        const double cc = p.d * xn / (double)od;
        NT_STORE(cc, &c.Tw[xi]);
        if (hub) __hip_atomic_store(&hub[GW + c.t], cc, __ATOMIC_RELAXED, __HIP_MEMORY_SCOPE_AGENT);
        else c.csum += cc;
        return;
    }
    if (c.act) {
        NT_STORE(xn, &p.x[xi]);
        if (!hub) c.dsum += fabs(xn - xo);
    } else {
        xn = xo;
    }
    double cc = 0.0;
    if (lrow < p.sl_nd) {
        cc = p.d * xn / (double)od;
        NT_STORE(cc, &c.Tw[xi]);
        if (!hub) c.csum += cc;
    }
    if (hub) {
        __hip_atomic_store(&hub[c.t], fabs(xn - xo), __ATOMIC_RELAXED, __HIP_MEMORY_SCOPE_AGENT);
        __hip_atomic_store(&hub[GW + c.t], cc, __ATOMIC_RELAXED, __HIP_MEMORY_SCOPE_AGENT);
    }
}

template <int GW, bool TS, bool LEAN>
__device__ __forceinline__ void long_rows(SweepCtx<GW, TS, LEAN>& c, const WorkItem* __restrict__ work, uint32_t i0, uint32_t i1, int lane) {
    constexpr int NS = 64 / GW;
    constexpr uint32_t TW = NS * CH;
    const PrParams& p = c.p;
    if (i0 >= i1) return;
    WorkItem cur = work[i0], nxt = work[i0 + 1];
    uint32_t src_n[CH / GW];
    {
        const uint32_t e0 = cur.beg + (uint32_t)c.slot * CH;
        idx_turn<GW>(p.in_src, e0, turn_fill(e0, cur.end), p.zrow, c.t, src_n);
    }
    for (uint32_t it = i0; it < i1; it++) {
        const WorkItem nn = work[it + 2];
        const uint32_t lrow = cur.row;
        double xo = 0.0;
        if constexpr (!LEAN) xo = NT_LOAD(&p.x[(size_t)lrow * GW + c.t]);
        const uint32_t od = lrow < p.sl_nd ? NT_LOAD(&p.outdeg[lrow]) : 1u;
        const uint32_t turns = (cur.end - cur.beg + TW - 1) / TW;
        const bool more = it + 1 < i1;
        double acc = 0.0;
        for (uint32_t i = 0; i < turns; i++) {
            uint32_t src[CH / GW];
#pragma unroll
            for (int r = 0; r < CH / GW; r++) src[r] = src_n[r];
            const bool last = i + 1 == turns;
            const uint32_t e1 = (last ? nxt.beg : cur.beg + (i + 1) * TW) + (uint32_t)c.slot * CH;
            const uint32_t lim = last ? (more ? nxt.end : 0u) : cur.end;
            idx_turn<GW>(p.in_src, e1, turn_fill(e1, lim), p.zrow, c.t, src_n);
            double v[CH];
            gather_turn<GW>(c.T, src, c.t, c.gbase, v);
#pragma unroll
            for (int j = 0; j < CH; j++) acc += v[j];
        }
        const double y = wave_sum_topic<GW>(acc);
        if (cur.kind == V_ROWW) {
            if (lane < GW) finish_row<GW>(c, lrow, y, xo, od);
        } else {
            if (lane < GW) __hip_atomic_store(&p.segpart[(size_t)(cur.sbase + cur.count) * GW + c.t], y, __ATOMIC_RELAXED, __HIP_MEMORY_SCOPE_AGENT);
            asm volatile("s_waitcnt vmcnt(0)" ::: "memory");
            unsigned prev = 0;
            if (lane == 0) prev = __hip_atomic_fetch_add(&p.rowticket[cur.tix], 1u, __ATOMIC_RELAXED, __HIP_MEMORY_SCOPE_AGENT);
            prev = (unsigned)__builtin_amdgcn_readfirstlane((int)prev);
            if (prev == cur.nseg - 1) {
                if (lane == 0) __hip_atomic_store(&p.rowticket[cur.tix], 0u, __ATOMIC_RELAXED, __HIP_MEMORY_SCOPE_AGENT);
                if (lane < GW) {
                    double ys = 0.0;
                    for (uint32_t q = 0; q < cur.nseg; q++)
                        ys += __hip_atomic_load(&p.segpart[(size_t)(cur.sbase + q) * GW + c.t], __ATOMIC_RELAXED, __HIP_MEMORY_SCOPE_AGENT);
                    finish_row<GW>(c, lrow, ys, xo, od, p.hubsum + (size_t)cur.tix * 2 * GW);
                }
            }
        }
        cur = nxt;
        nxt = nn;
    }
}

template <int GW, bool TS, bool LEAN>
__device__ __forceinline__ void quad_rows(SweepCtx<GW, TS, LEAN>& c, const WorkItem* __restrict__ work, uint32_t i0, uint32_t i1) {
    constexpr int NS = 64 / GW;
    const PrParams& p = c.p;
    if (i0 >= i1) return;
    const uint32_t myq = (uint32_t)c.t * NS + (uint32_t)c.slot;
    auto bounds = [&](const WorkItem& w, bool live, uint32_t& bv, uint32_t& ev, uint32_t& ov) __attribute__((always_inline)) {
        const bool have = live && myq < w.count;
        const uint32_t rq = live ? w.row + (have ? myq : 0u) : 0u;
        const uint32_t b = p.in_ptr[rq], e = p.in_ptr[rq + 1];
        bv = b;
        ev = have ? e : b;
        ov = rq < p.sl_nd ? NT_LOAD(&p.outdeg[rq]) : 1u;
    };
    WorkItem cur = work[i0], nxt = work[i0 + 1];
    uint32_t cb, ce, co, nb, ne, no;
    bounds(cur, true, cb, ce, co);
    bounds(nxt, i0 + 1 < i1, nb, ne, no);
    uint32_t it = i0, q = 0, ch = 0;
    uint32_t nq = (cur.count + NS - 1) / NS, nch = cur.nseg;
    uint32_t src_n[CH / GW];
    {
        const uint32_t b0 = (uint32_t)__shfl((int)cb, c.gbase, 64), e0 = (uint32_t)__shfl((int)ce, c.gbase, 64);
        idx_turn<GW>(p.in_src, b0, turn_fill(b0, e0), p.zrow, c.t, src_n);
    }
    double acc = 0.0;
    while (it < i1) {
        uint32_t src[CH / GW];
#pragma unroll
        for (int r = 0; r < CH / GW; r++) src[r] = src_n[r];
        uint32_t qn = q, cn = ch + 1;
        bool cross = false;
        if (cn == nch) {
            cn = 0;
            qn = q + 1;
            if (qn == nq) { qn = 0; cross = true; }
        }
        const bool live_n = !cross || it + 1 < i1;
        {
            const uint32_t b_n = (uint32_t)__shfl((int)(cross ? nb : cb), c.gbase + (int)qn, 64);
            const uint32_t e_n = (uint32_t)__shfl((int)(cross ? ne : ce), c.gbase + (int)qn, 64);
            const uint32_t ep = b_n + cn * CH;
            idx_turn<GW>(p.in_src, ep, live_n ? turn_fill(ep, e_n) : 0u, p.zrow, c.t, src_n);
        }
        const bool ends = ch + 1 == nch;
        const uint32_t lrow = cur.row + q * NS + (uint32_t)c.slot;
        const bool valid = q * NS + (uint32_t)c.slot < cur.count;
        double xo = 0.0;
        if constexpr (!LEAN)
            if (ends) xo = NT_LOAD(&p.x[(size_t)(valid ? lrow : cur.row) * GW + c.t]);
        double v[CH];
        gather_turn<GW>(c.T, src, c.t, c.gbase, v);
#pragma unroll
        for (int j = 0; j < CH; j++) acc += v[j];
        if (ends) {
            const uint32_t od = (uint32_t)__shfl((int)co, c.gbase + (int)q, 64);
            if (valid) finish_row<GW>(c, lrow, acc, xo, od);
            acc = 0.0;
        }
        q = qn;
        ch = cn;
        if (cross) {
            it++;
            cur = nxt;
            cb = nb; ce = ne; co = no;
            nq = (cur.count + NS - 1) / NS;
            nch = cur.nseg;
            nxt = work[it + 1];
            bounds(nxt, it + 1 < i1, nb, ne, no);
        }
    }
}

template <int GW, int R, bool TS, bool LEAN>
__device__ __forceinline__ void deg_rows(SweepCtx<GW, TS, LEAN>& c, const WorkItem* __restrict__ work, uint32_t i0, uint32_t i1) {
    constexpr int NS = 64 / GW;
    constexpr int DM = CH / R;
    constexpr int IR = CH / GW;
    const PrParams& p = c.p;
    if (i0 >= i1) return;
    auto idx = [&](const WorkItem& w, bool live, uint32_t turn, uint32_t (&src)[IR]) __attribute__((always_inline)) {
        const uint32_t rb = (turn * NS + (uint32_t)c.slot) * R;
#pragma unroll
        for (int r = 0; r < IR; r++) {
            const uint32_t j = (uint32_t)(r * GW + c.t);
            const uint32_t rr = rb + j / DM, u = j % DM;
            const bool ok = live && u < w.nseg && rr < w.count;
            const uint32_t raw = NT_LOAD(&p.in_src[ok ? w.beg + rr * w.nseg + u : 0u]);
            src[r] = ok ? (raw & SRC_MASK) : p.zrow;
        }
    };
    WorkItem cur = work[i0], nxt = work[i0 + 1];
    uint32_t src_n[IR];
    idx(cur, true, 0, src_n);
    for (uint32_t it = i0; it < i1; it++) {
        const WorkItem nn = work[it + 2];
        const uint32_t row0 = cur.row, count = cur.count;
        const uint32_t turns = (count + NS * R - 1) / (NS * R);
        for (uint32_t i = 0; i < turns; i++) {
            uint32_t src[IR];
#pragma unroll
            for (int r = 0; r < IR; r++) src[r] = src_n[r];
            if (i + 1 < turns) idx(cur, true, i + 1, src_n);
            else idx(nxt, it + 1 < i1, 0, src_n);
            const uint32_t rb = (i * NS + (uint32_t)c.slot) * R;
            double xo[R];
#pragma unroll
            for (int r = 0; r < R; r++) {
                xo[r] = 0.0;
                if constexpr (!LEAN) xo[r] = NT_LOAD(&p.x[(size_t)(row0 + (rb + r < count ? rb + r : 0u)) * GW + c.t]);
            }
            const uint32_t myr = row0 + (rb + (uint32_t)c.t < count ? rb + (uint32_t)c.t : 0u);
            const uint32_t odv = (c.t < R && myr < p.sl_nd) ? NT_LOAD(&p.outdeg[myr]) : 1u;
            double v[CH];
            gather_turn<GW>(c.T, src, c.t, c.gbase, v);
#pragma unroll
            for (int r = 0; r < R; r++) {
                double y = 0.0;
#pragma unroll
                for (int u = 0; u < DM; u++) y += v[r * DM + u];
                const uint32_t od = (uint32_t)__shfl((int)odv, c.gbase + r, 64);
                if (rb + r < count) finish_row<GW>(c, row0 + rb + r, y, xo[r], od);
            }
        }
        cur = nxt;
        nxt = nn;
    }
}

#ifndef SS_PR_MINW
#define SS_PR_MINW 1
#endif
#ifdef SS_PR_WAVETIME
__device__ unsigned long long g_pr_wt[65536][2];
#endif
template <int GW, bool TS, bool LEAN>
__global__ __launch_bounds__(TPB, SS_PR_MINW) void k_pr_sweep(PrParams p) {
    static_assert(!(TS && LEAN), "the lean sweep exists without teleport sets only");
    constexpr int NS = 64 / GW;
    PrCtl* ctl = p.ctl;
    if (ctl->n_active == 0) return;
#ifdef SS_PR_WAVETIME
    unsigned long long wt0;
    asm volatile("s_memrealtime %0\n\ts_waitcnt lgkmcnt(0)" : "=s"(wt0));
#endif
    const int sweep = ctl->sweep;
    const int lane = threadIdx.x & 63;
    const uint32_t wave = (uint32_t)__builtin_amdgcn_readfirstlane((int)(threadIdx.x >> 6));
    SweepCtx<GW, TS, LEAN> c{p, p.tab_rd[sweep & 1], p.tab_wr[sweep & 1], 0.0, 0.0, false, lane % GW, lane - lane % GW, lane / GW, 0.0, 0.0};
    c.S = ctl->S[c.t];
    c.act = ctl->active[c.t] != 0;
    c.x0 = sweep == 0 ? p.x0[c.t] : 0.0;

    if constexpr (!TS) {
        if (p.n_shared) {
            const double xz_out = c.act ? zero_row_rank(p, sweep, c.S, p.x0[c.t]) : ctl->xz[c.t];
            const uint32_t nel = p.n_shared * (uint32_t)GW;
            for (uint32_t i = blockIdx.x * TPB + threadIdx.x; i < nel; i += gridDim.x * TPB)
                c.Tw[(size_t)(p.zrow + 1) * GW + i] = p.d * xz_out / (double)p.sh_deg[i / GW];
        }
    }

    const uint32_t* __restrict__ off = (LEAN ? p.woff_lean : p.woff) + (size_t)(blockIdx.x * WAVES + wave) * 8;
    int rot = p.stagger_div ? (int)((blockIdx.x / p.stagger_div) % 6u) : 0;
    if (p.stagger_code) {
        uint32_t cdv = p.stagger_code;
        for (uint32_t r = blockIdx.x / p.stagger_div; r > 0; r--) cdv /= 6u;
        rot = (int)(cdv % 6u);
    }
    for (int s6 = 0; s6 < 6; s6++) {
    const int cls = (int)((p.class_order >> (3 * ((s6 + rot) % 6))) & 7u);
    {
        int ln = lane;
        asm volatile("" : "+v"(ln));
        c.t = ln % GW;
        c.gbase = ln - ln % GW;
        c.slot = ln / GW;
    }
    switch (cls) {
    case 0: long_rows<GW>(c, p.work, off[0], off[1], lane); break;
    case 1: quad_rows<GW>(c, p.work, off[1], off[2]); break;
    case 2: deg_rows<GW, 2>(c, p.work, off[2], off[3]); break;
    case 3: deg_rows<GW, 4>(c, p.work, off[3], off[4]); break;
    case 4: deg_rows<GW, 8>(c, p.work, off[4], off[5]); break;
    default:
    for (uint32_t item = off[5]; item < off[6]; item++) {
        const WorkItem w = p.work[item];
        const bool store = TS || !p.share;
        const bool ts = TS && p.memb && ((p.ts_mask >> c.t) & 1u);
        const double xz_out = c.act ? (ts ? zero_row_rank_ts(p, sweep, c.S, p.x0[c.t], 0.0) : zero_row_rank(p, sweep, c.S, p.x0[c.t])) : ctl->xz[c.t];
        const double xz_inn = ts ? (c.act ? zero_row_rank_ts(p, sweep, c.S, p.x0[c.t], p.tin[c.t]) : ctl->xz_in[c.t]) : xz_out;
        uint32_t od[16];
#pragma unroll
        for (int i = 0; i < 16; i++) {
            const uint32_t rr = (uint32_t)(i * NS + c.slot);
            od[i] = NT_LOAD(&p.outdeg[w.row + (rr < w.count ? rr : 0u)]);
        }
#pragma unroll
        for (int i = 0; i < 16; i++) {
            const uint32_t rr = (uint32_t)(i * NS + c.slot);
            if (rr < w.count) {
                const uint32_t lrow = w.row + rr;
                const double xz = ts && ((p.memb[lrow] >> c.t) & 1u) ? xz_inn : xz_out;
                const double cc = p.d * xz / (double)od[i];
                if (store) NT_STORE(cc, &c.Tw[(size_t)lrow * GW + c.t]);
                c.csum += cc;
            }
        }
    }
    break;
    }
    }
#ifdef SS_PR_WAVETIME
    {
        unsigned long long wt1;
        asm volatile("s_waitcnt vmcnt(0)\n\ts_memrealtime %0\n\ts_waitcnt lgkmcnt(0)" : "=s"(wt1));
        const uint32_t wid = (blockIdx.x * WAVES + wave) & 65535u;
        if (lane == 0) { g_pr_wt[wid][0] = wt0; g_pr_wt[wid][1] = wt1; }
    }
#endif
    block_reduce_and_publish<GW>(p, LEAN ? 0.0 : c.dsum, c.csum, c.Tw, false);
}

template __device__ void begin_caller_context<8, 16>(const PrParams&, double*);

}

namespace ss {
void pr_sweep_launch(ss_pr* pr, hipStream_t st, bool lean) {
    const bool ts = pr->prm.memb != nullptr;
    lean = lean && !ts && pr->prm.woff_lean;
    if (lean) pr->n_lean++;
    if (pr->gw == 8) {
        if (ts) hipLaunchKernelGGL((k_pr_sweep<8, true, false>), dim3(pr->nblocks), dim3(TPB), 0, st, pr->prm);
        else if (lean) hipLaunchKernelGGL((k_pr_sweep<8, false, true>), dim3(pr->nblocks), dim3(TPB), 0, st, pr->prm);
        else hipLaunchKernelGGL((k_pr_sweep<8, false, false>), dim3(pr->nblocks), dim3(TPB), 0, st, pr->prm);
    } else {
        if (ts) hipLaunchKernelGGL((k_pr_sweep<16, true, false>), dim3(pr->nblocks), dim3(TPB), 0, st, pr->prm);
        else if (lean) hipLaunchKernelGGL((k_pr_sweep<16, false, true>), dim3(pr->nblocks), dim3(TPB), 0, st, pr->prm);
        else hipLaunchKernelGGL((k_pr_sweep<16, false, false>), dim3(pr->nblocks), dim3(TPB), 0, st, pr->prm);
    }
}
int pr_sweep_occupancy(int gw) {
    int per_cu = 8;
    if (gw == 8) (void)hipOccupancyMaxActiveBlocksPerMultiprocessor(&per_cu, k_pr_sweep<8, false, false>, TPB, 0);
    else (void)hipOccupancyMaxActiveBlocksPerMultiprocessor(&per_cu, k_pr_sweep<16, false, false>, TPB, 0);
    return per_cu;
}

#ifdef SS_PR_WAVETIME
void pr_dump_wave_times(const ss_pr* pr) {
    if (pr->gw < 8) return;
    (void)hipDeviceSynchronize();
    const uint32_t nwv = std::min<uint32_t>(65536u, pr->nblocks * WAVES);
    std::vector<unsigned long long> h((size_t)nwv * 2);
    if (hipMemcpyFromSymbol(h.data(), HIP_SYMBOL(g_pr_wt), h.size() * sizeof(unsigned long long)) != hipSuccess || !nwv) return;
    unsigned long long t0 = ~0ull;
    for (uint32_t w = 0; w < nwv; w++) t0 = std::min(t0, h[2 * w]);
    std::vector<double> st(nwv), en(nwv);
    for (uint32_t w = 0; w < nwv; w++) { st[w] = (double)(h[2 * w] - t0) / 100.0; en[w] = (double)(h[2 * w + 1] - t0) / 100.0; }
    std::sort(st.begin(), st.end()); std::sort(en.begin(), en.end());
    if (FILE* f = open_dump("pr_wt.csv")) {
        fprintf(f, "wave,start_us,end_us\n");
        for (uint32_t w = 0; w < nwv; w++) fprintf(f, "%u,%.2f,%.2f\n", w, (double)(h[2 * w] - t0) / 100.0, (double)(h[2 * w + 1] - t0) / 100.0);
        fclose(f);
    }
    fprintf(stderr, "[pr wavetime] %u waves: start us median %.1f max %.1f | out of items us min %.1f p10 %.1f median %.1f p90 %.1f p99 %.1f max %.1f\n", nwv,
            st[nwv / 2], st[nwv - 1], en[0], en[nwv / 10], en[nwv / 2], en[nwv * 9 / 10], en[(size_t)nwv * 99 / 100], en[nwv - 1]);
}
#endif
}
```

### spaghettisearch_amd/engine.py

```python
from __future__ import annotations

import ctypes as C
from typing import Optional, Sequence

import numpy as np

from . import _lib
from ._lib import SsGraphInfo, SsHit, SsPassage, SsTermMatch, check

HIT_DTYPE = np.dtype([("doc", "<u4"), ("_pad", "<u4"), ("title", "<f8"), ("body", "<f8"),
                      ("pagerank", "<f8"), ("final", "<f8")])

TERM_MATCH_DTYPE = np.dtype([("title_w", "<f4"), ("body_w", "<f4"), ("flags", "<u4"), ("body_pos", "<f4")])

PASSAGE_DTYPE = np.dtype([("start", "<f4"), ("last", "<f4"), ("n_distinct", "<u4"), ("n_occ", "<u4"), ("token_mask", "<u8")])

DOC_RANGE_DTYPE = np.dtype([("field", "<i4"), ("_pad", "<i4"), ("lo", "<i8"), ("hi", "<i8")])

VEC_HIT_DTYPE = np.dtype([("doc", "<u4"), ("score", "<i4")])

GROUP_COUNT_DTYPE = np.dtype([("group", "<u4"), ("count", "<u4")])

DIV_INFO_DTYPE = np.dtype([("rel", "<i4"), ("sim", "<i4")])

# ... 159 lines not shown
    def apply_delta(self, n_nodes_new: int, changed, new_ptr, new_children) -> None:
        changed = _as(changed, "uint32")
        new_ptr = _as(new_ptr, "uint64")
        new_children = _as(new_children, "uint32")
        self.ctx.ready(changed, new_ptr, new_children)
        check(self.ctx.lib.ss_graph_apply_delta(self.h, int(n_nodes_new), int(changed.shape[0]), _ptr(changed), _ptr(new_ptr), _ptr(new_children)),
              self.ctx.h)
        self.n = int(n_nodes_new)

    def info(self) -> SsGraphInfo:
        gi = SsGraphInfo()
        check(self.ctx.lib.ss_graph_get_info(self.h, C.byref(gi)), self.ctx.h)
        return gi

    def pagerank_sharded(self, damping: float, eps: float, n_topic: Sequence[int], max_iter: int = 0, allreduce: bool = False, out=None):
        n_topic = np.ascontiguousarray(np.atleast_1d(n_topic), dtype=np.int32)
        K = len(n_topic)
        rows = int(self.info().n_rows_local)
        if out is not None:
            ids, rank = _as(out[0], "uint32"), _as(out[1], "float64")
            count = lambda a: a.numel() if _is_torch(a) else a.size
            if count(ids) < rows or count(rank) < K * rows:
                raise ValueError("out arrays too small")
        else:
            ids = np.zeros(rows, dtype=np.uint32)
            rank = np.zeros((K, rows), dtype=np.float64)
        iters = np.zeros(K, dtype=np.int32)
        check(self.ctx.lib.ss_pagerank_run_sharded(self.h, damping, eps, max_iter, K, _ptr(n_topic), 1 if allreduce else 0,
                                                   _ptr(ids), _ptr(rank), _ptr(iters)), self.ctx.h)
        return ids, rank, iters

    def pagerank(self, damping: float, eps: float, n_topic: Sequence[int], max_iter: int = 0):
        n_topic = np.ascontiguousarray(np.atleast_1d(n_topic), dtype=np.int32)
        K = len(n_topic)
        rank = np.zeros((K, self.n), dtype=np.float64)
        iters = np.zeros(K, dtype=np.int32)
        check(self.ctx.lib.ss_pagerank_run(self.h, damping, eps, max_iter, K, _ptr(n_topic), _ptr(rank), _ptr(iters)),
              self.ctx.h)
        return rank, iters

    @staticmethod
    def pagerank_group(shards, damping: float, eps: float, n_topic: Sequence[int], max_iter: int = 0):
        n_topic = np.ascontiguousarray(np.atleast_1d(n_topic), dtype=np.int32)
        K = len(n_topic)
        ctx = shards[0].ctx
        hs = (C.c_void_p * len(shards))(*[g.h for g in shards])
        rank = np.zeros((K, shards[0].n), dtype=np.float64)
        iters = np.zeros(K, dtype=np.int32)
        check(ctx.lib.ss_pagerank_run_group(hs, len(shards), damping, eps, max_iter, K, _ptr(n_topic), _ptr(rank), _ptr(iters)), ctx.h)
        return rank, iters

    def pagerank_dev(self, damping: float, eps: float, n_topic: Sequence[int], rank_out, max_iter: int = 0):
        n_topic = np.ascontiguousarray(np.atleast_1d(n_topic), dtype=np.int32)
        K = len(n_topic)
        rank_out = _as(rank_out, "float64")
        if rank_out.numel() < K * self.n:
            raise ValueError("rank_out too small")
        iters = np.zeros(K, dtype=np.int32)
        check(self.ctx.lib.ss_pagerank_run(self.h, damping, eps, max_iter, K, _ptr(n_topic), _ptr(rank_out), _ptr(iters)),
              self.ctx.h)
        return iters

    def set_link_key(self, key) -> None:
        if key is None:
            check(self.ctx.lib.ss_graph_set_link_key(self.h, None), self.ctx.h)
            return
        key = _as(key, "float64")
        if (key.numel() if _is_torch(key) else key.size) < self.n:
            raise ValueError("key must hold n_nodes values")
        self.ctx.ready(key)
        check(self.ctx.lib.ss_graph_set_link_key(self.h, _ptr(key)), self.ctx.h)

    def _links_out(self, rows: int, m: int, want_degree: bool, out):
        count = lambda a: a.numel() if _is_torch(a) else a.size
        if out is not None:
            links, n_out, degree = _as(out[0], "uint32"), _as(out[1], "int32"), _as(out[2], "uint32") if len(out) > 2 else None
            if count(links) < rows * m or count(n_out) < rows or (degree is not None and count(degree) < rows):
                raise ValueError("output buffers too small")
            return links, n_out, degree
        return np.zeros(rows * m, dtype=np.uint32), np.zeros(rows, dtype=np.int32), np.zeros(rows, dtype=np.uint32) if want_degree else None

    def top_links(self, nodes, direction: int, m: int = 5, want_degree: bool = True, out=None):
        nodes = _as(nodes, "uint32")
        n = int(nodes.numel() if _is_torch(nodes) else nodes.size)
        links, n_out, degree = self._links_out(n, int(m), want_degree, out)
        self.ctx.ready(nodes, links, n_out, degree)
        check(self.ctx.lib.ss_graph_top_links(self.h, int(direction), n, _ptr(nodes), int(m), _ptr(links), _ptr(n_out), _ptr(degree)), self.ctx.h)
        if out is None:
            links = links.reshape(n, int(m))
        elif any(_is_torch(a) for a in (links, n_out, degree)) and not getattr(self.ctx, "_shared_stream", False):
            self.ctx.synchronize()
        return links, n_out, degree

    def hit_links(self, hits, n_hits, direction: int, m: int = 5, want_degree: bool = True, out=None, k: Optional[int] = None):
        n_hits = _as(n_hits, "int32")
        n_q = int(n_hits.numel() if _is_torch(n_hits) else n_hits.size)
        nbytes = lambda a: a.numel() * a.element_size() if _is_torch(a) else a.nbytes
        hits = hits.contiguous() if _is_torch(hits) else np.ascontiguousarray(hits, dtype=HIT_DTYPE)
        if k is None:
            if n_q > 0 and nbytes(hits) % (n_q * HIT_DTYPE.itemsize):
                raise ValueError("hits does not hold n_q rows of whole ss_hit")
            k = nbytes(hits) // (n_q * HIT_DTYPE.itemsize) if n_q > 0 else 1
        elif nbytes(hits) < n_q * int(k) * HIT_DTYPE.itemsize:
            raise ValueError("hits too small")
        k = int(k)
        links, n_out, degree = self._links_out(n_q * k, int(m), want_degree, out)
        self.ctx.ready(hits, n_hits, links, n_out, degree)
        check(self.ctx.lib.ss_graph_hit_links(self.h, int(direction), n_q, k, _ptr(hits), _ptr(n_hits), int(m), _ptr(links), _ptr(n_out),
                                              _ptr(degree)), self.ctx.h)
        if out is None:
            links, n_out = links.reshape(n_q, k, int(m)), n_out.reshape(n_q, k)
            degree = degree.reshape(n_q, k) if degree is not None else None
        elif any(_is_torch(a) for a in (links, n_out, degree)) and not getattr(self.ctx, "_shared_stream", False):
            self.ctx.synchronize()
        return links, n_out, degree

    def close(self) -> None:
        if self.h:
            self.ctx.lib.ss_graph_destroy(self.h)
            self.h = None


class PageRankState:

    def __init__(self, graph: Graph, damping: float, eps: float, n_topic: Sequence[int], max_iter: int = 0):
        self.g = graph
        self.ctx = graph.ctx
        n_topic = np.ascontiguousarray(np.atleast_1d(n_topic), dtype=np.int32)
        self.k = len(n_topic)
        h = C.c_void_p()
        check(self.ctx.lib.ss_pr_create(graph.h, damping, eps, max_iter, self.k, _ptr(n_topic), C.byref(h)), self.ctx.h)
        self.h = h

    def set_teleport(self, sets) -> None:
        if sets is None:
            check(self.ctx.lib.ss_pr_set_teleport(self.h, None, None), self.ctx.h)
            return
        if len(sets) != self.k:
            raise ValueError("one teleport set per topic")
        ptr = np.zeros(self.k + 1, dtype=np.uint64)
        ptr[1:] = np.cumsum([len(x) for x in sets])
        nodes = np.ascontiguousarray(np.concatenate([np.asarray(x, dtype=np.uint32) for x in sets]) if int(ptr[-1]) else np.zeros(0, np.uint32))
        check(self.ctx.lib.ss_pr_set_teleport(self.h, _ptr(ptr), _ptr(nodes)), self.ctx.h)

    def begin(self) -> None:
        check(self.ctx.lib.ss_pr_begin(self.h), self.ctx.h)

    def step(self, n_steps: int = 1) -> None:
        check(self.ctx.lib.ss_pr_step(self.h, n_steps), self.ctx.h)

    def lean_sweeps(self) -> int:
        n = C.c_int64(0)
        check(self.ctx.lib.ss_pr_lean_sweeps(self.h, C.byref(n)), self.ctx.h)
        return int(n.value)

    def finalize(self) -> None:
        check(self.ctx.lib.ss_pr_finalize(self.h), self.ctx.h)

    def exchange(self, allreduce: bool = False) -> None:
        check(self.ctx.lib.ss_pr_exchange(self.h, 1 if allreduce else 0), self.ctx.h)

    def exchange_buffers(self):
        sp, rp = C.c_void_p(), C.c_void_p()
        sb, rb = C.c_uint64(), C.c_uint64()
        check(self.ctx.lib.ss_pr_exchange_buffers(self.h, C.byref(sp), C.byref(sb), C.byref(rp), C.byref(rb)), self.ctx.h)
        return sp.value, sb.value, rp.value, rb.value

    def status(self):
        iters = np.zeros(self.k, dtype=np.int32)
        delta = np.zeros(self.k, dtype=np.float64)
        total = np.zeros(self.k, dtype=np.float64)
        na, sw = C.c_int32(), C.c_int32()
        check(self.ctx.lib.ss_pr_status(self.h, _ptr(iters), C.byref(na), C.byref(sw), _ptr(delta), _ptr(total)), self.ctx.h)
        return {"iters": iters, "n_active": na.value, "sweeps": sw.value, "delta": delta, "total": total}

    def probe(self, mode: int = 0, n_reps: int = 5) -> float:
        ms = C.c_float(0)
        check(self.ctx.lib.ss_pr_probe(self.h, mode, n_reps, C.byref(ms)), self.ctx.h)
        return float(ms.value)

    def read(self) -> np.ndarray:
        out = np.zeros((self.k, self.g.n), dtype=np.float64)
        check(self.ctx.lib.ss_pr_read(self.h, _ptr(out)), self.ctx.h)
        return out

    def read_local(self):
        n_rows = int(self.g.info().n_rows_local)
        ids = np.zeros(n_rows, dtype=np.uint32)
        out = np.zeros((self.k, n_rows), dtype=np.float64)
        check(self.ctx.lib.ss_pr_read_local(self.h, _ptr(ids), _ptr(out)), self.ctx.h)
        return ids, out

    def close(self) -> None:
        if self.h:
            self.ctx.lib.ss_pr_destroy(self.h)
            self.h = None


class InvertedIndex:

    def __init__(self, ctx: Context, n_docs: int, term_ptr, post_doc, post_tf):
        self.ctx = ctx
        self.n_docs = int(n_docs)
        term_ptr = _as(term_ptr, "uint64")
        post_doc = _as(post_doc, "uint32")
        post_tf = _as(post_tf, "float32")
        self.n_terms = int(term_ptr.shape[0]) - 1
        self.n_post = int(post_doc.shape[0])
        ctx.ready(term_ptr, post_doc, post_tf)
        h = C.c_void_p()
        check(ctx.lib.ss_index_create(ctx.h, self.n_docs, self.n_terms, _ptr(term_ptr), _ptr(post_doc), _ptr(post_tf),
                                      C.byref(h)), ctx.h)
        self.h = h

    def tfidf_build(self, total_docs: int, want_w: bool = True, want_mag: bool = True, want_idf: bool = True):
        w = np.zeros(self.n_post, dtype=np.float32) if want_w else None
        mag = np.zeros(self.n_docs, dtype=np.float64) if want_mag else None
        idf = np.zeros(self.n_terms, dtype=np.float32) if want_idf else None
        check(self.ctx.lib.ss_tfidf_build(self.h, int(total_docs), _ptr(w), _ptr(mag), _ptr(idf)), self.ctx.h)
        return w, mag, idf

    def apply_delta(self, del_docs=None, del_pairs=None, add=None, add_pos=None) -> None:
        dd = _as(del_docs if del_docs is not None else np.zeros(0, np.uint32), "uint32")
        dt, dp = (_as(del_pairs[0], "uint32"), _as(del_pairs[1], "uint32")) if del_pairs is not None else (np.zeros(0, np.uint32),) * 2
        at, ad, aw = (_as(add[0], "uint32"), _as(add[1], "uint32"), _as(add[2], "float32")) if add is not None else \
            (np.zeros(0, np.uint32), np.zeros(0, np.uint32), np.zeros(0, np.float32))
        pp, pv = (_as(add_pos[0], "uint64"), _as(add_pos[1], "float32")) if add_pos is not None else (None, None)
        self.ctx.ready(dd, dt, dp, at, ad, aw, pp, pv)
        check(self.ctx.lib.ss_index_apply_delta_pos(self.h, int(dd.shape[0]), _ptr(dd), int(dt.shape[0]), _ptr(dt), _ptr(dp),
                                                    int(at.shape[0]), _ptr(at), _ptr(ad), _ptr(aw), _ptr(pp), _ptr(pv)), self.ctx.h)
        n_post = C.c_uint64()
        check(self.ctx.lib.ss_index_get_info(self.h, None, None, C.byref(n_post)), self.ctx.h)
        self.n_post = int(n_post.value)

    def resize(self, n_docs: int, n_terms: int) -> None:
        check(self.ctx.lib.ss_index_resize(self.h, int(n_docs), int(n_terms)), self.ctx.h)
        self.n_docs, self.n_terms = int(n_docs), int(n_terms)

    def read_magnitudes(self, docs) -> np.ndarray:
        docs = _as(docs, "uint32")
        out = np.zeros(int(docs.shape[0]), dtype=np.float64)
        check(self.ctx.lib.ss_index_read_magnitudes(self.h, int(docs.shape[0]), _ptr(docs), _ptr(out)), self.ctx.h)
        return out

    def read_positions(self):
        pp = np.zeros(self.n_post + 1, dtype=np.uint64)
        check(self.ctx.lib.ss_index_read_positions(self.h, _ptr(pp), None), self.ctx.h)
        pv = np.zeros(int(pp[-1]), dtype=np.float32)
        check(self.ctx.lib.ss_index_read_positions(self.h, None, _ptr(pv)), self.ctx.h)
        return pp, pv

    def refresh_magnitudes(self) -> np.ndarray:
        mag = np.zeros(self.n_docs, dtype=np.float64)
        check(self.ctx.lib.ss_index_refresh_magnitudes(self.h, _ptr(mag)), self.ctx.h)
        return mag

    def read(self):
        tp = np.zeros(self.n_terms + 1, dtype=np.uint64)
        pd = np.zeros(self.n_post, dtype=np.uint32)
        pw = np.zeros(self.n_post, dtype=np.float32)
        check(self.ctx.lib.ss_index_read(self.h, _ptr(tp), _ptr(pd), _ptr(pw)), self.ctx.h)
        return tp, pd, pw

    def build_doc_view(self) -> None:
        check(self.ctx.lib.ss_index_build_doc_view(self.h), self.ctx.h)

    def drop_doc_view(self) -> None:
        check(self.ctx.lib.ss_index_drop_doc_view(self.h), self.ctx.h)

    def read_doc_view(self):
        dp = np.zeros(self.n_docs + 1, dtype=np.uint64)
        check(self.ctx.lib.ss_index_read_doc_view(self.h, _ptr(dp), None, None), self.ctx.h)
        dt = np.zeros(int(dp[-1]), dtype=np.uint32)
        dw = np.zeros(int(dp[-1]), dtype=np.float32)
        check(self.ctx.lib.ss_index_read_doc_view(self.h, None, _ptr(dt), _ptr(dw)), self.ctx.h)
        return dp, dt, dw

    def doc_top_terms(self, docs, m: int, want_w: bool = True, out=None):
        docs = _as(docs, "uint32")
        n = int(docs.shape[0])
        if out is not None:
            terms, w, n_out = _as(out[0], "uint32"), _as(out[1], "float32"), _as(out[2], "int32")
            count = lambda a: a.numel() if _is_torch(a) else a.size
            if count(terms) < n * m or (w is not None and count(w) < n * m) or count(n_out) < n:
                raise ValueError("output buffers too small")
        else:
            terms = np.zeros((n, m), dtype=np.uint32)
            w = np.zeros((n, m), dtype=np.float32) if want_w else None
            n_out = np.zeros(n, dtype=np.int32)
        self.ctx.ready(docs, terms, w, n_out)
        check(self.ctx.lib.ss_index_doc_top_terms(self.h, n, _ptr(docs), int(m), _ptr(terms), _ptr(w), _ptr(n_out)), self.ctx.h)
        return terms, w, n_out

    def build_signatures(self, n_slots: int = 16) -> None:
        check(self.ctx.lib.ss_index_build_signatures(self.h, int(n_slots)), self.ctx.h)

    def drop_signatures(self) -> None:
        check(self.ctx.lib.ss_index_drop_signatures(self.h), self.ctx.h)

    def read_signatures(self, docs, out=None):
        docs = _as(docs, "uint32")
        n = int(docs.numel() if _is_torch(docs) else docs.size)
        n_slots = C.c_int32(0)
        check(self.ctx.lib.ss_index_read_signatures(self.h, 0, None, None, C.byref(n_slots)), self.ctx.h)
        if out is None:
            out = np.zeros((n, n_slots.value), dtype=np.uint32)
# ... 957 lines not shown
```

Baseline: 21140.

## Add hand-in block publish and store-only sweep mode for PageRank

Adds a new block_publish_one path in which each block writes its partial sums to a grouped hand-in layout. The last block, found by a ticket counter, reduces everything and updates the control state inside the same sweep kernel, replacing the earlier block_reduce_and_publish path. It also adds a PR_STORE sweep mode that writes x but skips reading old x and the delta sum, used for non-final steps when a lean sweep cannot be used. The work-offset load is hoisted ahead of the n_active check, and the shared zero-row fill moves to the end of the kernel. Together these aim to cut reduction, synchronisation and memory traffic per iteration, at the cost of a serial final-block reduction and extra code complexity.

```diff
diff --git a/include/spaghetti_rank.h b/include/spaghetti_rank.h
--- a/include/spaghetti_rank.h
+++ b/include/spaghetti_rank.h
@@ -99,6 +99,7 @@
 int32_t ss_pr_begin(ss_pr* pr);
 int32_t ss_pr_step(ss_pr* pr, int32_t n_steps);
 int32_t ss_pr_lean_sweeps(ss_pr* pr, int64_t* n_out);
+int32_t ss_pr_store_sweeps(ss_pr* pr, int64_t* n_out);
 int32_t ss_pr_finalize(ss_pr* pr);
 int32_t ss_pr_exchange_buffers(ss_pr* pr, void** send_dev, uint64_t* send_bytes,
                                void** recv_dev, uint64_t* recv_bytes);
diff --git a/spaghettisearch_amd/_lib.py b/spaghettisearch_amd/_lib.py
--- a/spaghettisearch_amd/_lib.py
+++ b/spaghettisearch_amd/_lib.py
@@ -117,6 +117,7 @@
     "ss_pr_begin": (_i32, [_vp]),
     "ss_pr_step": (_i32, [_vp, _i32]),
     "ss_pr_lean_sweeps": (_i32, [_vp, C.POINTER(C.c_int64)]),
+    "ss_pr_store_sweeps": (_i32, [_vp, C.POINTER(C.c_int64)]),
     "ss_pr_finalize": (_i32, [_vp]),
     "ss_pr_exchange_buffers": (_i32, [_vp, C.POINTER(_vp), C.POINTER(_u64), C.POINTER(_vp), C.POINTER(_u64)]),
     "ss_pr_exchange": (_i32, [_vp, _i32]),
diff --git a/spaghettisearch_amd/csrc/ctx.hip b/spaghettisearch_amd/csrc/ctx.hip
--- a/spaghettisearch_amd/csrc/ctx.hip
+++ b/spaghettisearch_amd/csrc/ctx.hip
@@ -281,6 +281,7 @@
     "pr.deal_global",
     "pr.share_zero_rows",
     "pr.lean_sweeps",
+    "pr.handin",
     "pr.item_turns",
     "graph.late_free",
     "graph.readback_runs",
diff --git a/spaghettisearch_amd/csrc/pagerank.hip b/spaghettisearch_amd/csrc/pagerank.hip
--- a/spaghettisearch_amd/csrc/pagerank.hip
+++ b/spaghettisearch_amd/csrc/pagerank.hip
@@ -272,10 +272,10 @@
 namespace ss {
 unsigned begin_blocks(const ss_pr* pr) { return std::max(1u, std::min(2048u, ss::div_up((size_t)pr->g->n_local() * pr->gw, TPB))); }
 void pr_launch_begin(ss_pr* pr, hipStream_t st, unsigned nb) { SS_GW_DISPATCH(pr->gw, launch_begin, pr, st, nb); }
-void pr_launch_step(ss_pr* pr, hipStream_t st, bool lean) {
+void pr_launch_step(ss_pr* pr, hipStream_t st, int mode) {
     switch (pr->kernel) {
         case PR_STEP: pr_step_launch(pr, st); break;
-        case PR_SWEEP: pr_sweep_launch(pr, st, lean); break;
+        case PR_SWEEP: pr_sweep_launch(pr, st, mode); break;
         case PR_SWEEP_N: pr_sweep_n_launch(pr, st); break;
     }
 }
@@ -542,7 +542,9 @@
         if (trace) fprintf(stderr, "[pr trace]   shared rows: %u rows without in-edges -> %zu shared rows (host %.3f ms), table %llu rows\n", n_tail, sh.deg.size(),
                            t_ms(ts0, ts1), (unsigned long long)sh.table_rows);
     }
-    SS_HIP(ctx, pr->partials.alloc(((size_t)std::max(pr->nblocks, ss::begin_blocks(pr)) + 8) * 2 * GW));
+    pr->prm.handin = pr->kernel == PR_SWEEP && g->world == 1 && ctx->opt("pr.affine", 0) == 0 && ctx->opt("pr.handin", 1) != 0 ? 1u : 0u;
+    SS_HIP(ctx, pr->partials.alloc(std::max(((size_t)std::max(pr->nblocks, ss::begin_blocks(pr)) + 8) * 2 * GW,
+                                            handin_doubles(pr->nblocks, GW))));
     SS_HIP(ctx, pr->segpart.alloc((size_t)std::max(cut.nsegs, 1u) * GW));
     SS_HIP(ctx, pr->rowticket.alloc(std::max(cut.nmulti, 1u)));
     SS_HIP(ctx, pr->hubsum.alloc((size_t)std::max(cut.nmulti, 1u) * 2 * GW));
@@ -710,6 +712,13 @@
     return SS_OK;
 }
 
+int32_t ss_pr_store_sweeps(ss_pr* pr, int64_t* n_out) {
+    if (!pr || !n_out) return SS_ERR_INVALID;
+    std::lock_guard<std::recursive_mutex> lk(pr->g->ctx->mu);
+    *n_out = pr->n_store;
+    return SS_OK;
+}
+
 }
 
 int32_t ss::pr_step(ss_pr* pr, int32_t n_steps, int32_t full_tail) {
@@ -729,7 +738,8 @@
         for (int i = 0; i < n_steps; i++) {
             const int64_t s = pr->sweeps_enq + 1 + i;
             const bool lean = lean_ok && i + full_tail < n_steps && (p.max_iter <= 0 || s + 2 <= p.max_iter);
-            ss::pr_launch_step(pr, ctx->stream, lean);
+            const bool read = (full_tail > 0 && i + 1 == n_steps) || (p.max_iter > 0 && s >= p.max_iter);
+            ss::pr_launch_step(pr, ctx->stream, lean ? PR_LEAN : lean_ok && !read ? PR_STORE : PR_FULL);
         }
     }
     pr->sweeps_enq += n_steps;
diff --git a/spaghettisearch_amd/csrc/pr_device.hpp b/spaghettisearch_amd/csrc/pr_device.hpp
--- a/spaghettisearch_amd/csrc/pr_device.hpp
+++ b/spaghettisearch_amd/csrc/pr_device.hpp
@@ -264,6 +264,138 @@
     }
 }
 
+template <int GW, bool CS_ONLY>
+__device__ __forceinline__ void block_publish_one(const PrParams& p, double dsum, double csum, double S_t, bool act_t, int sweep) {
+    constexpr int NCOL = 2 * GW;
+    constexpr int NPART = TPB / NCOL;
+    __shared__ double red[WAVES][2][MAXK];
+    __shared__ double gsum[HANDIN_NG][TPB];
+    __shared__ double hsum[TPB];
+    __shared__ double tot[2][MAXK];
+    __shared__ int s_last;
+    const int lane = threadIdx.x & 63, wave = threadIdx.x >> 6;
+    if constexpr (!CS_ONLY) dsum = wave_sum_topic<GW>(dsum);
+    csum = wave_sum_topic<GW>(csum);
+    if (lane < GW) {
+        if constexpr (!CS_ONLY) red[wave][0][lane] = dsum;
+        red[wave][1][lane] = csum;
+    }
+    __syncthreads();
+    const bool mine = threadIdx.x < NCOL && (!CS_ONLY || threadIdx.x >= GW);
+    if (mine) {
+        const int which = threadIdx.x / GW, tt = threadIdx.x % GW;
+        double v = red[0][which][tt];
+#pragma unroll
+        for (int w = 1; w < WAVES; w++) v += red[w][which][tt];
+        __hip_atomic_store(&p.partials[(size_t)handin_row(blockIdx.x, gridDim.x, NPART) * NCOL + threadIdx.x], v, __ATOMIC_RELAXED, __HIP_MEMORY_SCOPE_AGENT);
+    }
+    asm volatile("s_waitcnt vmcnt(0)" ::: "memory");
+    __syncthreads();
+    if (threadIdx.x == 0) {
+        const unsigned prev = __hip_atomic_fetch_add(&p.ctl->ticket, 1u, __ATOMIC_RELAXED, __HIP_MEMORY_SCOPE_AGENT);
+        s_last = prev == gridDim.x - 1;
+    }
+    __syncthreads();
+    if (!s_last) return;
+    const int col = threadIdx.x % NCOL, part = threadIdx.x / NCOL;
+    const bool rd = !CS_ONLY || col >= GW;
+    const int k = threadIdx.x;
+    const bool ts = p.memb && k < GW && ((p.ts_mask >> k) & 1u);
+    double xz_old = 0.0, xz_in_old = 0.0;
+    if (!CS_ONLY && k < GW) {
+        xz_old = p.ctl->xz[k];
+        if (ts) xz_in_old = p.ctl->xz_in[k];
+    }
+    const uint32_t ng = handin_groups(gridDim.x), turns = handin_turns(gridDim.x, NPART);
+    for (uint32_t g0 = 0; g0 < ng; g0 += 2) {
+        double acc[2] = {0.0, 0.0};
+        uint32_t members[2];
+#pragma unroll
+        for (int h = 0; h < 2; h++) members[h] = g0 + h < ng ? handin_members(gridDim.x, g0 + h) : 0u;
+        for (uint32_t u0 = 0; u0 < turns; u0 += 16) {
+            double v[2][16];
+#pragma unroll
+            for (int h = 0; h < 2; h++)
+#pragma unroll
+                for (int u = 0; u < 16; u++) {
+                    const bool ok = rd && (uint32_t)part + (u0 + u) * NPART < members[h];
+                    const size_t tile = ok ? (size_t)(g0 + h) * turns + u0 + u : 0u;
+                    v[h][u] = __hip_atomic_load(&p.partials[tile * TPB + threadIdx.x], __ATOMIC_RELAXED, __HIP_MEMORY_SCOPE_AGENT);
+                }
+#pragma unroll
+            for (int h = 0; h < 2; h++)
+#pragma unroll
+                for (int u = 0; u < 16; u++)
+                    if ((uint32_t)part + (u0 + u) * NPART < members[h]) acc[h] += v[h][u];
+        }
+        gsum[g0][threadIdx.x] = acc[0];
+        if (g0 + 1 < ng) gsum[g0 + 1][threadIdx.x] = acc[1];
+    }
+    if (p.nmulti && part > 0 && rd) {
+        const unsigned hp = part - 1;
+        double acc = 0.0;
+        for (unsigned h0 = hp; h0 < p.nmulti; h0 += 16 * (NPART - 1)) {
+            double v[16];
+#pragma unroll
+            for (int u = 0; u < 16; u++) {
+                const unsigned h = h0 + u * (NPART - 1);
+                v[u] = __hip_atomic_load(&p.hubsum[(size_t)(h < p.nmulti ? h : h0) * NCOL + col], __ATOMIC_RELAXED, __HIP_MEMORY_SCOPE_AGENT);
+            }
+#pragma unroll
+            for (int u = 0; u < 16; u++)
+                if (h0 + u * (NPART - 1) < p.nmulti) acc += v[u];
+        }
+        hsum[threadIdx.x] = acc;
+    }
+    __syncthreads();
+    if (threadIdx.x < NCOL) {
+        double v = 0.0;
+        if (rd) {
+            for (uint32_t g = 0; g < ng; g++) {
+                double gv = 0.0;
+#pragma unroll
+                for (int q = 0; q < NPART; q++) gv += gsum[g][q * NCOL + threadIdx.x];
+                v += gv;
+            }
+            if (p.nmulti)
+                for (int q = 1; q < NPART; q++) v += hsum[q * NCOL + threadIdx.x];
+        }
+        tot[threadIdx.x / GW][threadIdx.x % GW] = v;
+    }
+    __syncthreads();
+    if (threadIdx.x >= 64) return;
+    const int it = sweep + 1;
+    bool cont = false;
+    if (k < p.k_topics && k < GW && act_t) {
+        double dl = 0.0;
+        const double xz = zero_row_rank(p, sweep, S_t, p.x0[k]);
+        const double xz_out = ts ? zero_row_rank_ts(p, sweep, S_t, p.x0[k], 0.0) : xz;
+        const double xz_in = ts ? zero_row_rank_ts(p, sweep, S_t, p.x0[k], p.tin[k]) : xz;
+        if constexpr (!CS_ONLY) {
+            const double n_zero = (double)((p.cnt_nd - p.pos_nd) + (p.cnt_d - p.pos_d));
+            dl = tot[0][k];
+            if (ts) dl += (n_zero - p.nz_in[k]) * fabs(xz_out - xz_old) + p.nz_in[k] * fabs(xz_in - xz_in_old);
+            else dl += n_zero * fabs(xz - xz_old);
+        }
+        const double cs = tot[1][k];
+        p.ctl->iters[k] = it;
+        p.ctl->delta[k] = dl;
+        p.ctl->xz[k] = xz_out;
+        p.ctl->xz_in[k] = xz_in;
+        cont = dl > p.eps;
+        if (p.max_iter > 0 && it >= p.max_iter) cont = false;
+        p.ctl->active[k] = cont ? 1 : 0;
+        p.ctl->S[k] = cs + p.tele_n;
+        p.ctl->csum[k] = cs;
+    }
+    const int na = __popcll(__ballot(cont));
+    if (threadIdx.x == 0) {
+        p.ctl->ticket = 0u;
+        p.ctl->n_active = na;
+        p.ctl->sweep = it;
+    }
+}
+
 template <int GA, int GB>
 __device__ __attribute__((used, noinline)) void begin_caller_context(const PrParams& p, double* tail) {
     if (!__builtin_constant_p(p.world)) return;
diff --git a/spaghettisearch_amd/csrc/pr_plan.hpp b/spaghettisearch_amd/csrc/pr_plan.hpp
--- a/spaghettisearch_amd/csrc/pr_plan.hpp
+++ b/spaghettisearch_amd/csrc/pr_plan.hpp
@@ -376,4 +376,18 @@
     return sh;
 }
 
-}
+constexpr uint32_t HANDIN_NG = 8;
+constexpr uint32_t handin_groups(uint32_t nblocks) { return nblocks < HANDIN_NG ? nblocks : HANDIN_NG; }
+constexpr uint32_t handin_members(uint32_t nblocks, uint32_t grp) {
+    return (nblocks - grp + handin_groups(nblocks) - 1) / handin_groups(nblocks);
+}
+constexpr uint32_t handin_turns(uint32_t nblocks, uint32_t npart) { return nblocks ? plan_div_up(handin_members(nblocks, 0), npart) : 0u; }
+constexpr uint32_t handin_row(uint32_t b, uint32_t nblocks, uint32_t npart) {
+    const uint32_t ng = handin_groups(nblocks), grp = b % ng, m = b / ng;
+    return ((grp * handin_turns(nblocks, npart) + m / npart) * npart) + m % npart;
+}
+constexpr size_t handin_doubles(uint32_t nblocks, int gw) {
+    return (size_t)handin_groups(nblocks) * handin_turns(nblocks, (uint32_t)(TPB / (2 * gw))) * TPB;
+}
+
+}
diff --git a/spaghettisearch_amd/csrc/pr_state.hpp b/spaghettisearch_amd/csrc/pr_state.hpp
--- a/spaghettisearch_amd/csrc/pr_state.hpp
+++ b/spaghettisearch_amd/csrc/pr_state.hpp
@@ -77,7 +77,10 @@
     uint32_t share;
     uint32_t tab_rows;
     const uint32_t* woff_lean;
+    uint32_t handin;
 };
+
+enum PrSweepMode : int { PR_FULL = 0, PR_LEAN = 1, PR_STORE = 2 };
 
 }
 
@@ -110,6 +113,7 @@
     bool lean = false;
     int64_t sweeps_enq = 0;
     int64_t n_lean = 0;
+    int64_t n_store = 0;
     ss::DevBuf<PrCtl> ctl;
     bool begun = false;
     bool need_finalize = false;
@@ -120,10 +124,10 @@
 namespace ss {
 unsigned begin_blocks(const ss_pr* pr);
 void pr_launch_begin(ss_pr* pr, hipStream_t st, unsigned nb);
-void pr_launch_step(ss_pr* pr, hipStream_t st, bool lean = false);
+void pr_launch_step(ss_pr* pr, hipStream_t st, int mode = PR_FULL);
 int32_t pr_step(ss_pr* pr, int32_t n_steps, int32_t full_tail);
 void pr_launch_finalize(ss_pr* pr, hipStream_t st, int is_begin);
-void pr_sweep_launch(ss_pr* pr, hipStream_t st, bool lean);
+void pr_sweep_launch(ss_pr* pr, hipStream_t st, int mode);
 int pr_sweep_occupancy(int gw);
 void pr_sweep_n_launch(ss_pr* pr, hipStream_t st);
 int pr_sweep_n_occupancy(int gw);
diff --git a/spaghettisearch_amd/csrc/pr_sweep.hip b/spaghettisearch_amd/csrc/pr_sweep.hip
--- a/spaghettisearch_amd/csrc/pr_sweep.hip
+++ b/spaghettisearch_amd/csrc/pr_sweep.hip
@@ -10,7 +10,7 @@
 }
 
 
-template <int GW, bool TS, bool LEAN>
+template <int GW, bool TS, int MODE>
 struct SweepCtx {
     const PrParams& p;
     const double* __restrict__ T;
@@ -43,15 +43,15 @@
     }
 }
 
-template <int GW, bool TS, bool LEAN>
-__device__ __forceinline__ void finish_row(SweepCtx<GW, TS, LEAN>& c, uint32_t lrow, double y, double xo, uint32_t od, double* hub = nullptr) {
+template <int GW, bool TS, int MODE>
+__device__ __forceinline__ void finish_row(SweepCtx<GW, TS, MODE>& c, uint32_t lrow, double y, double xo, uint32_t od, double* hub = nullptr) {
     const PrParams& p = c.p;
     y += c.x0;
     const size_t xi = (size_t)lrow * GW + c.t;
     double tele = p.teleport;
     if constexpr (TS) tele = teleport_of(p, lrow, c.t);
     double xn = (y + tele) / c.S;
-    if constexpr (LEAN) {
+    if constexpr (MODE == PR_LEAN) {
         if (!c.act) xn = 0.0;
         const double cc = p.d * xn / (double)od;
         NT_STORE(cc, &c.Tw[xi]);
@@ -59,6 +59,18 @@
         else c.csum += cc;
         return;
     }
+    if constexpr (MODE == PR_STORE) {
+        if (c.act) NT_STORE(xn, &p.x[xi]);
+        else xn = 0.0;
+        double cc = 0.0;
+        if (lrow < p.sl_nd) {
+            cc = p.d * xn / (double)od;
+            NT_STORE(cc, &c.Tw[xi]);
+            if (!hub) c.csum += cc;
+        }
+        if (hub) __hip_atomic_store(&hub[GW + c.t], cc, __ATOMIC_RELAXED, __HIP_MEMORY_SCOPE_AGENT);
+        return;
+    }
     if (c.act) {
         NT_STORE(xn, &p.x[xi]);
         if (!hub) c.dsum += fabs(xn - xo);
@@ -77,8 +89,8 @@
     }
 }
 
-template <int GW, bool TS, bool LEAN>
-__device__ __forceinline__ void long_rows(SweepCtx<GW, TS, LEAN>& c, const WorkItem* __restrict__ work, uint32_t i0, uint32_t i1, int lane) {
+template <int GW, bool TS, int MODE>
+__device__ __forceinline__ void long_rows(SweepCtx<GW, TS, MODE>& c, const WorkItem* __restrict__ work, uint32_t i0, uint32_t i1, int lane) {
     constexpr int NS = 64 / GW;
     constexpr uint32_t TW = NS * CH;
     const PrParams& p = c.p;
@@ -93,7 +105,7 @@
         const WorkItem nn = work[it + 2];
         const uint32_t lrow = cur.row;
         double xo = 0.0;
-        if constexpr (!LEAN) xo = NT_LOAD(&p.x[(size_t)lrow * GW + c.t]);
+        if constexpr (MODE == PR_FULL) xo = NT_LOAD(&p.x[(size_t)lrow * GW + c.t]);
         const uint32_t od = lrow < p.sl_nd ? NT_LOAD(&p.outdeg[lrow]) : 1u;
         const uint32_t turns = (cur.end - cur.beg + TW - 1) / TW;
         const bool more = it + 1 < i1;
@@ -135,8 +147,8 @@
     }
 }
 
-template <int GW, bool TS, bool LEAN>
-__device__ __forceinline__ void quad_rows(SweepCtx<GW, TS, LEAN>& c, const WorkItem* __restrict__ work, uint32_t i0, uint32_t i1) {
+template <int GW, bool TS, int MODE>
+__device__ __forceinline__ void quad_rows(SweepCtx<GW, TS, MODE>& c, const WorkItem* __restrict__ work, uint32_t i0, uint32_t i1) {
     constexpr int NS = 64 / GW;
     const PrParams& p = c.p;
     if (i0 >= i1) return;
@@ -183,7 +195,7 @@
         const uint32_t lrow = cur.row + q * NS + (uint32_t)c.slot;
         const bool valid = q * NS + (uint32_t)c.slot < cur.count;
         double xo = 0.0;
-        if constexpr (!LEAN)
+        if constexpr (MODE == PR_FULL)
             if (ends) xo = NT_LOAD(&p.x[(size_t)(valid ? lrow : cur.row) * GW + c.t]);
         double v[CH];
         gather_turn<GW>(c.T, src, c.t, c.gbase, v);
@@ -208,8 +220,8 @@
     }
 }
 
-template <int GW, int R, bool TS, bool LEAN>
-__device__ __forceinline__ void deg_rows(SweepCtx<GW, TS, LEAN>& c, const WorkItem* __restrict__ work, uint32_t i0, uint32_t i1) {
+template <int GW, int R, bool TS, int MODE>
+__device__ __forceinline__ void deg_rows(SweepCtx<GW, TS, MODE>& c, const WorkItem* __restrict__ work, uint32_t i0, uint32_t i1) {
     constexpr int NS = 64 / GW;
     constexpr int DM = CH / R;
     constexpr int IR = CH / GW;
@@ -244,7 +256,7 @@
 #pragma unroll
             for (int r = 0; r < R; r++) {
                 xo[r] = 0.0;
-                if constexpr (!LEAN) xo[r] = NT_LOAD(&p.x[(size_t)(row0 + (rb + r < count ? rb + r : 0u)) * GW + c.t]);
+                if constexpr (MODE == PR_FULL) xo[r] = NT_LOAD(&p.x[(size_t)(row0 + (rb + r < count ? rb + r : 0u)) * GW + c.t]);
             }
             const uint32_t myr = row0 + (rb + (uint32_t)c.t < count ? rb + (uint32_t)c.t : 0u);
             const uint32_t odv = (c.t < R && myr < p.sl_nd) ? NT_LOAD(&p.outdeg[myr]) : 1u;
@@ -270,34 +282,28 @@
 #ifdef SS_PR_WAVETIME
 __device__ unsigned long long g_pr_wt[65536][2];
 #endif
-template <int GW, bool TS, bool LEAN>
+template <int GW, bool TS, int MODE>
 __global__ __launch_bounds__(TPB, SS_PR_MINW) void k_pr_sweep(PrParams p) {
-    static_assert(!(TS && LEAN), "the lean sweep exists without teleport sets only");
+    static_assert(!(TS && MODE != PR_FULL), "the lean and the store-only sweep exist without teleport sets only");
     constexpr int NS = 64 / GW;
     PrCtl* ctl = p.ctl;
-    if (ctl->n_active == 0) return;
+    const uint32_t wave = (uint32_t)__builtin_amdgcn_readfirstlane((int)(threadIdx.x >> 6));
+    const uint32_t* __restrict__ offp = (MODE == PR_LEAN ? p.woff_lean : p.woff) + (size_t)(blockIdx.x * WAVES + wave) * 8;
+    uint32_t off[7];
+#pragma unroll
+    for (int i = 0; i < 7; i++) off[i] = offp[i];
+    const int n_active = ctl->n_active, sweep = ctl->sweep;
+    if (n_active == 0) return;
 #ifdef SS_PR_WAVETIME
     unsigned long long wt0;
     asm volatile("s_memrealtime %0\n\ts_waitcnt lgkmcnt(0)" : "=s"(wt0));
 #endif
-    const int sweep = ctl->sweep;
     const int lane = threadIdx.x & 63;
-    const uint32_t wave = (uint32_t)__builtin_amdgcn_readfirstlane((int)(threadIdx.x >> 6));
-    SweepCtx<GW, TS, LEAN> c{p, p.tab_rd[sweep & 1], p.tab_wr[sweep & 1], 0.0, 0.0, false, lane % GW, lane - lane % GW, lane / GW, 0.0, 0.0};
+    SweepCtx<GW, TS, MODE> c{p, p.tab_rd[sweep & 1], p.tab_wr[sweep & 1], 0.0, 0.0, false, lane % GW, lane - lane % GW, lane / GW, 0.0, 0.0};
     c.S = ctl->S[c.t];
     c.act = ctl->active[c.t] != 0;
     c.x0 = sweep == 0 ? p.x0[c.t] : 0.0;
 
-    if constexpr (!TS) {
-        if (p.n_shared) {
-            const double xz_out = c.act ? zero_row_rank(p, sweep, c.S, p.x0[c.t]) : ctl->xz[c.t];
-            const uint32_t nel = p.n_shared * (uint32_t)GW;
-            for (uint32_t i = blockIdx.x * TPB + threadIdx.x; i < nel; i += gridDim.x * TPB)
-                c.Tw[(size_t)(p.zrow + 1) * GW + i] = p.d * xz_out / (double)p.sh_deg[i / GW];
-        }
-    }
-
-    const uint32_t* __restrict__ off = (LEAN ? p.woff_lean : p.woff) + (size_t)(blockIdx.x * WAVES + wave) * 8;
     int rot = p.stagger_div ? (int)((blockIdx.x / p.stagger_div) % 6u) : 0;
     if (p.stagger_code) {
         uint32_t cdv = p.stagger_code;
@@ -347,6 +353,14 @@
     break;
     }
     }
+    if constexpr (!TS) {
+        const uint32_t nel = p.n_shared * (uint32_t)GW;
+        if (blockIdx.x * TPB + threadIdx.x < nel) {
+            const double xz_out = c.act ? zero_row_rank(p, sweep, c.S, p.x0[c.t]) : ctl->xz[c.t];
+            for (uint32_t i = blockIdx.x * TPB + threadIdx.x; i < nel; i += gridDim.x * TPB)
+                c.Tw[(size_t)(p.zrow + 1) * GW + i] = p.d * xz_out / (double)p.sh_deg[i / GW];
+        }
+    }
 #ifdef SS_PR_WAVETIME
     {
         unsigned long long wt1;
@@ -355,7 +369,8 @@
         if (lane == 0) { g_pr_wt[wid][0] = wt0; g_pr_wt[wid][1] = wt1; }
     }
 #endif
-    block_reduce_and_publish<GW>(p, LEAN ? 0.0 : c.dsum, c.csum, c.Tw, false);
+    if (p.handin) block_publish_one<GW, MODE != PR_FULL>(p, c.dsum, c.csum, c.S, c.act, sweep);
+    else block_reduce_and_publish<GW>(p, MODE == PR_FULL ? c.dsum : 0.0, c.csum, c.Tw, false);
 }
 
 template __device__ void begin_caller_context<8, 16>(const PrParams&, double*);
@@ -363,24 +378,27 @@
 }
 
 namespace ss {
-void pr_sweep_launch(ss_pr* pr, hipStream_t st, bool lean) {
+void pr_sweep_launch(ss_pr* pr, hipStream_t st, int mode) {
     const bool ts = pr->prm.memb != nullptr;
-    lean = lean && !ts && pr->prm.woff_lean;
-    if (lean) pr->n_lean++;
+    if (ts || !pr->prm.woff_lean) mode = PR_FULL;
+    if (mode == PR_LEAN) pr->n_lean++;
+    if (mode == PR_STORE) pr->n_store++;
     if (pr->gw == 8) {
-        if (ts) hipLaunchKernelGGL((k_pr_sweep<8, true, false>), dim3(pr->nblocks), dim3(TPB), 0, st, pr->prm);
-        else if (lean) hipLaunchKernelGGL((k_pr_sweep<8, false, true>), dim3(pr->nblocks), dim3(TPB), 0, st, pr->prm);
-        else hipLaunchKernelGGL((k_pr_sweep<8, false, false>), dim3(pr->nblocks), dim3(TPB), 0, st, pr->prm);
+        if (ts) hipLaunchKernelGGL((k_pr_sweep<8, true, PR_FULL>), dim3(pr->nblocks), dim3(TPB), 0, st, pr->prm);
+        else if (mode == PR_LEAN) hipLaunchKernelGGL((k_pr_sweep<8, false, PR_LEAN>), dim3(pr->nblocks), dim3(TPB), 0, st, pr->prm);
+        else if (mode == PR_STORE) hipLaunchKernelGGL((k_pr_sweep<8, false, PR_STORE>), dim3(pr->nblocks), dim3(TPB), 0, st, pr->prm);
+        else hipLaunchKernelGGL((k_pr_sweep<8, false, PR_FULL>), dim3(pr->nblocks), dim3(TPB), 0, st, pr->prm);
     } else {
-        if (ts) hipLaunchKernelGGL((k_pr_sweep<16, true, false>), dim3(pr->nblocks), dim3(TPB), 0, st, pr->prm);
-        else if (lean) hipLaunchKernelGGL((k_pr_sweep<16, false, true>), dim3(pr->nblocks), dim3(TPB), 0, st, pr->prm);
-        else hipLaunchKernelGGL((k_pr_sweep<16, false, false>), dim3(pr->nblocks), dim3(TPB), 0, st, pr->prm);
+        if (ts) hipLaunchKernelGGL((k_pr_sweep<16, true, PR_FULL>), dim3(pr->nblocks), dim3(TPB), 0, st, pr->prm);
+        else if (mode == PR_LEAN) hipLaunchKernelGGL((k_pr_sweep<16, false, PR_LEAN>), dim3(pr->nblocks), dim3(TPB), 0, st, pr->prm);
+        else if (mode == PR_STORE) hipLaunchKernelGGL((k_pr_sweep<16, false, PR_STORE>), dim3(pr->nblocks), dim3(TPB), 0, st, pr->prm);
+        else hipLaunchKernelGGL((k_pr_sweep<16, false, PR_FULL>), dim3(pr->nblocks), dim3(TPB), 0, st, pr->prm);
     }
 }
 int pr_sweep_occupancy(int gw) {
     int per_cu = 8;
-    if (gw == 8) (void)hipOccupancyMaxActiveBlocksPerMultiprocessor(&per_cu, k_pr_sweep<8, false, false>, TPB, 0);
-    else (void)hipOccupancyMaxActiveBlocksPerMultiprocessor(&per_cu, k_pr_sweep<16, false, false>, TPB, 0);
+    if (gw == 8) (void)hipOccupancyMaxActiveBlocksPerMultiprocessor(&per_cu, k_pr_sweep<8, false, PR_FULL>, TPB, 0);
+    else (void)hipOccupancyMaxActiveBlocksPerMultiprocessor(&per_cu, k_pr_sweep<16, false, PR_FULL>, TPB, 0);
     return per_cu;
 }
 
diff --git a/spaghettisearch_amd/engine.py b/spaghettisearch_amd/engine.py
--- a/spaghettisearch_amd/engine.py
+++ b/spaghettisearch_amd/engine.py
@@ -335,6 +335,11 @@
     def lean_sweeps(self) -> int:
         n = C.c_int64(0)
         check(self.ctx.lib.ss_pr_lean_sweeps(self.h, C.byref(n)), self.ctx.h)
+        return int(n.value)
+
+    def store_sweeps(self) -> int:
+        n = C.c_int64(0)
+        check(self.ctx.lib.ss_pr_store_sweeps(self.h, C.byref(n)), self.ctx.h)
         return int(n.value)
 
     def finalize(self) -> None:
```

Result: no change. 21310, median of 6 (+0.8%).
